# fims9000/SYNT_ISIC

Hardware: AMD Instinct MI355X
Metric: images/sec at 3x64x64 T=1000 (DDPM reverse-diffusion sampling) (higher is better)
Workload: dtype f32

## Files before the change

synt_isic_amd/csrc/common.h:

```cpp
#pragma once

#include <hip/hip_runtime.h>

#include <atomic>
#include <cstdarg>
#include <cstdint>
#include <cstdio>
#include <string>
#include <map>
#include <mutex>
#include <vector>

#include "../../include/sisic.h"

namespace sisic {

void set_error(const char* fmt, ...);

#define SISIC_HIP(call)                                                                   \
    do {                                                                                  \
        hipError_t _e = (call);                                                           \
        if (_e != hipSuccess) {                                                           \
            ::sisic::set_error("%s failed: %s (%s:%d)", #call, hipGetErrorString(_e),     \
                               __FILE__, __LINE__);                                       \
            return SISIC_EHIP;                                                            \
        }                                                                                 \
    } while (0)

#define SISIC_REQUIRE(cond, ...)                 \
    do {                                         \
        if (!(cond)) {                           \
            ::sisic::set_error(__VA_ARGS__);     \
            return SISIC_EINVAL;                 \
        }                                        \
    } while (0)

#define SISIC_TRY(expr)             \
    do {                            \
        int _rc = (expr);           \
        if (_rc != SISIC_OK) return _rc; \
    } while (0)

enum ProfileKind { PK_CONV3 = 0, PK_CONV1 = 1, PK_GN = 2, PK_ATTN = 3, PK_DDPM = 4, PK_OTHER = 5, PK_WINO_MAIN = 6, PK_WINO_BF3 = 7, PK_COUNT = 8 };

struct ProfileSlot {
    double ms = 0, bytes = 0, flops = 0, flops_exec = 0;
    int64_t launches = 0;
};

struct PendingEvent {
    hipEvent_t start, stop;
    int kind;
    int kind2;
};

}

struct sisic_ctx {
    int device = 0;
    int num_cus = 0;
    bool profiling = false;
    sisic::ProfileSlot prof[sisic::PK_COUNT];
    std::vector<sisic::PendingEvent> pending;
    std::vector<hipEvent_t> event_pool;
    struct SplitK { float* p = nullptr; size_t floats = 0; };
    std::map<hipStream_t, SplitK> splitk;
    std::mutex splitk_mutex;
    std::atomic<uint64_t> scratch_generation{0};
};

namespace sisic {

struct ProfileScope {
    sisic_ctx* ctx;
    hipStream_t stream;
    PendingEvent ev{};
    bool active = false;
    ProfileScope(sisic_ctx* c, hipStream_t s, int kind, double bytes, double flops, double flops_exec = -1.0, int kind2 = -1);
    ~ProfileScope();
};

int profile_collect(sisic_ctx* ctx);

inline int ensure_dynamic_lds(sisic_ctx* ctx, const void* kern, int bytes, std::atomic<uint64_t>& done) {
    const uint64_t bit = uint64_t(1) << (ctx->device & 63);
    if (done.load(std::memory_order_acquire) & bit) return SISIC_OK;
    SISIC_HIP(hipFuncSetAttribute(kern, hipFuncAttributeMaxDynamicSharedMemorySize, bytes));
    done.fetch_or(bit, std::memory_order_release);
    return SISIC_OK;
}

inline int cdiv(int a, int b) { return (a + b - 1) / b; }
inline int wino_latency_ksplit(int Cout, int Cin, int Hout, int Wout) {
    const int co_t = Cout > 64 ? 128 : 64;
    const int per_image = cdiv(Hout, 8) * cdiv(Wout, 16) * cdiv(Cout, co_t);
    const int nchunks = cdiv(Cin, 8);
    int k = 1;
    while (per_image * k < 256 && k < 8 && nchunks % (2 * k) == 0) k *= 2;
    return k;
}
inline int wino_latency_segments(int Hout, int Wout) { return cdiv(Hout * Wout, 1024); }
inline int64_t cdiv64(int64_t a, int64_t b) { return (a + b - 1) / b; }
inline int round_up(int a, int b) { return cdiv(a, b) * b; }

constexpr int CONV_CO_TILE = 64;
inline int conv_ci_chunk(int ksize) { return ksize == 1 ? 32 : (ksize == 3 ? 16 : 4); }
inline int conv_cin_pad(int cin, int ksize) { return round_up(cin, conv_ci_chunk(ksize)); }
inline int conv_cout_pad(int cout) { return round_up(cout, CONV_CO_TILE); }
inline int64_t conv_packed_floats(int cout, int cin, int ksize) {
    const int64_t first = (int64_t)conv_cin_pad(cin, ksize) * ksize * ksize * conv_cout_pad(cout);
    return ksize == 1 ? 3 * first + first / 2 : first;
}

int launch_conv2d(sisic_ctx*, const sisic_conv_args& a, hipStream_t s);
int launch_conv_smallcout(sisic_ctx*, const sisic_conv_args& a, hipStream_t s);
int launch_score_head_bwd(sisic_ctx*, const float* logits, const float* fc_w, const float* act, float* g, int B, int C,
                          int HW, int n_classes, int target, hipStream_t s);
int launch_relu_bwd(sisic_ctx*, const float* dy, const float* y, float* out, int64_t n, hipStream_t s);
int launch_scatter_add_even(sisic_ctx*, float* dst, const float* src, int planes, int H, int W, hipStream_t s);
int launch_maxpool_bwd(sisic_ctx*, const float* dm, const float* xin, float* dx, int planes, int H, int W, hipStream_t s);
int launch_stem_bwd(sisic_ctx*, const float* g, const float* w_oihw, float* dp, int B, int CO, int OH, int OW, int H, int W,
                    hipStream_t s);
int launch_preprocess_bwd(sisic_ctx*, const float* dp, const float* x, float* dx, int B, int H, int W, int OH, int OW,
                          hipStream_t s);
int launch_add_relu(sisic_ctx*, const float* y, const float* identity, float* out, int64_t n, hipStream_t s);
int launch_gradcam(sisic_ctx*, const float* y, const float* outp, const float* fc_w, const float* bias, float* cam, int B, int C,
                   int h, int w, int S, int target, hipStream_t s);
int conv_stats_slots(const sisic_conv_args& a);
bool conv_finalizes(const sisic_conv_args& a);
bool conv_pointwise_applicable(const sisic_conv_args& a);
int conv_pointwise_stats_slots(const sisic_conv_args& a);
int launch_conv_pointwise(sisic_ctx*, const sisic_conv_args& a, hipStream_t s);
bool conv_pointwise_bf3_applicable(const sisic_conv_args& a);
int launch_conv_pointwise_bf3(sisic_ctx*, const sisic_conv_args& a, hipStream_t s);
int launch_gn_finalize(sisic_ctx*, const float* st0, int c0, int slots0, const float* st1, int c1, int slots1, int B,
                       int HW, int groups, float eps, const float* gamma, const float* beta, float* scale, float* shift,
                       hipStream_t s, float* mean_rstd = nullptr);
int launch_conv_winograd(sisic_ctx*, const sisic_conv_args& a, const float* u_packed, int cfg, hipStream_t s);
int launch_winograd_pack(sisic_ctx*, const float* w, int Cout, int Cin, float* packed, hipStream_t s);
int64_t winograd_packed_numel(int Cout, int Cin);
inline int64_t winograd_first_floats(int Cout, int Cin) { return (int64_t)round_up(Cin, 16) * 16 * conv_cout_pad(Cout); }
int launch_conv_pack(sisic_ctx*, const float* w, int Cout, int Cin, int k, float* packed, hipStream_t s);
int launch_gn_stats(sisic_ctx*, const float* in0, int c0, const float* in1, int c1, int B, int HW, int groups,
                    float eps, const float* gamma, const float* beta, float* scale, float* shift, hipStream_t s,
                    float* mean_rstd = nullptr);
int launch_attention(sisic_ctx*, const float* qkv, float* out, int B, int C, int N, int head_dim, hipStream_t s);
int launch_ddpm_step(sisic_ctx*, const float* eps, const float* x, const float* z, float* out, int64_t n,
                     float sb, float sa, float c0, float c1, float sigma, float clip, hipStream_t s);
size_t loop_state_bytes();
int launch_loop_select_row(sisic_ctx*, const float* table, int R, const void* state, float* out, hipStream_t s);
int launch_loop_advance(sisic_ctx*, void* state, hipStream_t s);
int launch_ddpm_step_indexed(sisic_ctx*, const float* eps, float* x, int64_t n, const void* state, const float* coef,
                             const int* zrow, float clip, hipStream_t s);
int launch_ddpm_step_rng(sisic_ctx*, const float* eps, const float* x, float* out, int64_t n, int64_t n_per_image,
                         const uint64_t* seeds_dev, uint32_t step, float sb, float sa, float c0, float c1, float sigma,
                         float clip, hipStream_t s);
int launch_ddpm_step_indexed_rng(sisic_ctx*, const float* eps, float* x, int64_t n, int64_t n_per_image, const void* state,
                                 const float* coef, const uint64_t* seeds_dev, float clip, hipStream_t s);
int launch_noise_fill(sisic_ctx*, void* out, int B, int64_t n_per_image, const uint64_t* seeds_host, uint32_t step,
                      uint32_t tag, bool bits, hipStream_t s);
int launch_denorm_u8(sisic_ctx*, const float* x, uint8_t* out, int B, int C, int H, int W, hipStream_t s, int form = 0);
int launch_temb_mlp(sisic_ctx*, const float* t_vals, int B, const float* freqs, int n_freqs, const float* w1t,
                    const float* b1, const float* w2t, const float* b2, int hidden, float* temb_act, hipStream_t s,
                    float* save_emb = nullptr, float* save_h1 = nullptr, float* save_t2 = nullptr);
int launch_linear_t(sisic_ctx*, const float* x, int B, int K, const float* wt, const float* bias, int R,
                    float* out, hipStream_t s);
int launch_transpose2d(sisic_ctx*, const float* in, int rows, int cols, float* out, int out_ld, int out_col0,
                       hipStream_t s);
int launch_preprocess(sisic_ctx*, const float* x, float* out, int B, int H, int W, int OH, int OW, hipStream_t s);
int launch_maxpool(sisic_ctx*, const float* x, float* out, int B, int C, int H, int W, hipStream_t s);
int launch_avgpool_fc(sisic_ctx*, const float* x, const float* w, const float* bias, float* out, int B, int C, int HW,
                      int n_out, hipStream_t s);
int launch_class_scores(sisic_ctx*, const float* logits, int B, int n, int target, float* prob, float* logscore,
                        hipStream_t s);
int launch_mask_patches(sisic_ctx*, const float* image, const uint8_t* masks, float* out, int S, int C, int H, int W,
                        int patch, hipStream_t s);

}
```

synt_isic_amd/csrc/conv_mfma.hip:

```cpp
#include <cstdlib>
#include <type_traits>

#include "common.h"
#include "pack_device.h"

namespace sisic {

typedef float f32x16 __attribute__((ext_vector_type(16)));

struct ConvParams {
    const float* in0;
    const float* in1;
    int c0, c1;
    int B, Hin, Win;
    int Hc, Wc;
    int Hout, Wout;
    int ups;
    int zero_insert;
    const float* w;
    int cout_pad;
    const float* bias;
    int Cout;
    const float* gn_scale;
    const float* gn_shift;
    int gn_silu;
    const float* chan_bias;
    int chan_bias_stride;
    const float* residual;
    int relu;
    float* out;
    float* stats;
    int* slots_query;
    int tiles_x, tiles_y, n_co_tiles, nwg, nchunks;
};

__device__ __forceinline__ float half_wave_sum(float v) {
    v += __int_as_float(__builtin_amdgcn_update_dpp(0, __float_as_int(v), 0xB1, 0xf, 0xf, true));
    v += __int_as_float(__builtin_amdgcn_update_dpp(0, __float_as_int(v), 0x4E, 0xf, 0xf, true));
    v += __int_as_float(__builtin_amdgcn_update_dpp(0, __float_as_int(v), 0x141, 0xf, 0xf, true));
    v += __int_as_float(__builtin_amdgcn_update_dpp(0, __float_as_int(v), 0x140, 0xf, 0xf, true));
    return v + __shfl_xor(v, 16);
}

__device__ __forceinline__ float silu_f(float v) { return v * __builtin_amdgcn_rcpf(1.0f + __expf(-v)); }

template <int KS, int STRIDE, int MT, int NT, int WM, int WN, int TW, int CIC, int KSP = 1>
struct ConvGeom {
    static constexpr int NWAVES = WM * WN * KSP;
    static constexpr int NTHR = 64 * NWAVES;
    static constexpr int CO_TILE = WM * MT * 32;
    static constexpr int PIX = WN * NT * 32;
    static constexpr int TH = PIX / TW;
    static constexpr int KK = KS * KS;
    static constexpr int PAD = KS / 2;
    static constexpr int IH = (TH - 1) * STRIDE + KS;
    static constexpr int IW = (TW - 1) * STRIDE + KS;
    static constexpr int TPC = NTHR / CIC;
    static constexpr int EPT = (IH * IW + TPC - 1) / TPC;
    static constexpr int CHS = EPT * TPC;
    static constexpr int IN_BUF = ((CIC * CHS + 3) / 4) * 4;
    static constexpr int W_F4 = CIC * KK * CO_TILE / 4;
    static constexpr int W_F4_PT = (W_F4 + NTHR - 1) / NTHR;
    static constexpr int W_BUF = W_F4_PT * NTHR * 4;
    static constexpr size_t LDS_BYTES = size_t(2) * (IN_BUF + W_BUF) * sizeof(float);
    static_assert(CO_TILE == CONV_CO_TILE, "weight packing assumes 64-channel tiles");
    static_assert(PIX % TW == 0, "tile must be whole rows");
    static_assert(NTHR % CIC == 0, "staging split");
    static_assert(CIC % (2 * KSP) == 0, "two channels per MFMA, whole pairs per K group");
};

template <int KS, int STRIDE, int MT, int NT, int WM, int WN, int TW, int CIC, int OCC, int KSP, bool V4 = false>
__global__ void __launch_bounds__(64 * WM * WN * KSP, OCC) conv_mfma_kernel(const ConvParams p) {
    using G = ConvGeom<KS, STRIDE, MT, NT, WM, WN, TW, CIC, KSP>;
    static_assert(!V4 || (KS == 1 && STRIDE == 1 && TW == G::PIX && G::EPT % 4 == 0 && G::CHS % 4 == 0),
                  "the float4 staging path is for flat 1x1 tiles");
    extern __shared__ __attribute__((aligned(16))) float smem[];
    float* const in_lds = smem;
    float* const w_lds = smem + 2 * G::IN_BUF;

    int work;
    {
        const int L = blockIdx.x, nwg = p.nwg;
        const int xcd = L & 7, slot = L >> 3, q = nwg >> 3, r = nwg & 7;
        work = (xcd < r ? xcd * (q + 1) : r * (q + 1) + (xcd - r) * q) + slot;
    }
    const int co_t = work % p.n_co_tiles;
    int tile = work / p.n_co_tiles;
    const int tx = tile % p.tiles_x;
    tile /= p.tiles_x;
    const int ty = tile % p.tiles_y;
    const int b = tile / p.tiles_y;
    const int oy0 = ty * G::TH, ox0 = tx * TW;
    const int co0 = co_t * G::CO_TILE;

    const int tid = threadIdx.x;
    const int lane = tid & 63;
    const int wave = tid >> 6;
    const int kg = wave / (WM * WN), wq = wave % (WM * WN);
    const int wm = wq / WN, wn = wq % WN;
    const int half = lane >> 5, l31 = lane & 31;

    const int sci = tid / G::TPC;
    const int sl = tid % G::TPC;
    const int HWin = p.Hin * p.Win;
    const int Cin = p.c0 + p.c1;
    int goff[G::EPT];
    unsigned vmask = 0;
    constexpr int EPT4 = V4 ? G::EPT / 4 : 1;
    int goff4[EPT4];
    unsigned vmask4 = 0;
    if constexpr (V4) {
#pragma unroll
        for (int i = 0; i < EPT4; ++i) {
            const int px = ox0 + 4 * sl + i * G::TPC * 4;
            const bool v = px < p.Wc;
            goff4[i] = v ? px : 0;
            vmask4 |= (v ? 1u : 0u) << i;
        }
    }
#pragma unroll
    for (int i = 0; i < (V4 ? 0 : G::EPT); ++i) {
        const int e = sl + i * G::TPC;
        const int yy = e / G::IW, xx = e % G::IW;
        const int gy = oy0 * STRIDE - G::PAD + yy;
        const int gx = ox0 * STRIDE - G::PAD + xx;
        const bool v = (e < G::IH * G::IW) && gy >= 0 && gy < p.Hc && gx >= 0 && gx < p.Wc &&
                       !(p.zero_insert && ((gy | gx) & 1));
        goff[i] = v ? ((gy >> p.ups) * p.Win + (gx >> p.ups)) : 0;
        vmask |= (v ? 1u : 0u) << i;
    }
    static_assert(G::EPT <= 32, "valid mask is 32 bits");

    const int a_base = half * G::KK * G::CO_TILE + wm * MT * 32 + l31;
    int b_base;
    {
        const int pix = wn * NT * 32 + l31;
        const int y = pix / TW, x = pix % TW;
        b_base = half * G::CHS + (y * STRIDE) * G::IW + x * STRIDE;
    }
    constexpr int NT_STEP = (TW >= 32) ? ((TW > 32) ? 32 * STRIDE : STRIDE * G::IW) : (32 / TW) * STRIDE * G::IW;
    static_assert(TW >= 32 || 32 % TW == 0, "TW must divide 32");
    static_assert(TW <= 32 || TW % 32 == 0, "TW must be a multiple of 32");

    f32x16 acc[MT][NT];
#pragma unroll
    for (int m = 0; m < MT; ++m)
#pragma unroll
        for (int n = 0; n < NT; ++n)
#pragma unroll
            for (int r = 0; r < 16; ++r) acc[m][n][r] = 0.0f;

    float rin[G::EPT];
    float rw[G::W_F4_PT * 4];
    float gsc = 1.0f, gsh = 0.0f;
    bool cval = false;

    const int prologue = (p.gn_scale == nullptr) ? 0 : (p.gn_silu ? 2 : 1);

    auto load_chunk = [&](int chunk) __attribute__((always_inline)) {
        const int c = chunk * CIC + sci;
        cval = c < Cin;
        const int cc = min(c, Cin - 1);
        const float* src = (cc < p.c0) ? p.in0 + ((size_t)b * p.c0 + cc) * HWin
                                       : p.in1 + ((size_t)b * p.c1 + (cc - p.c0)) * HWin;
        if constexpr (V4) {
#pragma unroll
            for (int i = 0; i < EPT4; ++i) {
                const float4 t = *reinterpret_cast<const float4*>(src + goff4[i]);
                rin[4 * i + 0] = t.x; rin[4 * i + 1] = t.y; rin[4 * i + 2] = t.z; rin[4 * i + 3] = t.w;
            }
        } else {
#pragma unroll
            for (int i = 0; i < G::EPT; ++i) rin[i] = src[goff[i]];
        }
        if (prologue) {
            gsc = p.gn_scale[(size_t)b * Cin + cc];
            gsh = p.gn_shift[(size_t)b * Cin + cc];
        }
        const float* wsrc = p.w + (size_t)chunk * CIC * G::KK * p.cout_pad + co0;
#pragma unroll
        for (int i = 0; i < G::W_F4_PT; ++i) {
            const int f = min(tid + i * G::NTHR, G::W_F4 - 1);
            const int rr = f / (G::CO_TILE / 4), c4 = f % (G::CO_TILE / 4);
            const float4 t = *reinterpret_cast<const float4*>(wsrc + (size_t)rr * p.cout_pad + c4 * 4);
            rw[4 * i + 0] = t.x; rw[4 * i + 1] = t.y; rw[4 * i + 2] = t.z; rw[4 * i + 3] = t.w;
        }
    };

    auto store_chunk = [&](const int buf) __attribute__((always_inline)) {
        float* dst = in_lds + buf * G::IN_BUF + sci * G::CHS + sl;
        const unsigned m = cval ? vmask : 0u;
        float v[G::EPT];
        if (prologue == 2) {
#pragma unroll
            for (int i = 0; i < G::EPT; ++i) v[i] = silu_f(rin[i] * gsc + gsh);
        } else if (prologue == 1) {
#pragma unroll
            for (int i = 0; i < G::EPT; ++i) v[i] = rin[i] * gsc + gsh;
        } else {
#pragma unroll
            for (int i = 0; i < G::EPT; ++i) v[i] = rin[i];
        }
        if constexpr (V4) {
            float* dst4 = in_lds + buf * G::IN_BUF + sci * G::CHS + 4 * sl;
            const unsigned m4 = cval ? vmask4 : 0u;
#pragma unroll
            for (int i = 0; i < EPT4; ++i) {
                const bool on = (m4 >> i) & 1u;
                *reinterpret_cast<float4*>(dst4 + i * G::TPC * 4) =
                    make_float4(on ? v[4 * i + 0] : 0.0f, on ? v[4 * i + 1] : 0.0f, on ? v[4 * i + 2] : 0.0f, on ? v[4 * i + 3] : 0.0f);
            }
        } else {
#pragma unroll
            for (int i = 0; i < G::EPT; ++i) dst[i * G::TPC] = ((m >> i) & 1u) ? v[i] : 0.0f;
        }
        float* wdst = w_lds + buf * G::W_BUF + tid * 4;
#pragma unroll
        for (int i = 0; i < G::W_F4_PT; ++i)
            *reinterpret_cast<float4*>(wdst + i * G::NTHR * 4) =
                make_float4(rw[4 * i + 0], rw[4 * i + 1], rw[4 * i + 2], rw[4 * i + 3]);
    };

    auto compute_chunk = [&](const int buf) __attribute__((always_inline)) {
        const float* A = w_lds + buf * G::W_BUF + a_base;
        const float* Bm = in_lds + buf * G::IN_BUF + b_base;
#pragma unroll
        for (int cp = kg * (CIC / 2 / KSP); cp < (kg + 1) * (CIC / 2 / KSP); ++cp) {
#pragma unroll
            for (int ky = 0; ky < KS; ++ky) {
#pragma unroll
                for (int kx = 0; kx < KS; ++kx) {
                    float a[MT], bb[NT];
#pragma unroll
                    for (int m = 0; m < MT; ++m)
                        a[m] = A[(2 * cp * G::KK + ky * KS + kx) * G::CO_TILE + m * 32];
#pragma unroll
                    for (int n = 0; n < NT; ++n)
                        bb[n] = Bm[2 * cp * G::CHS + ky * G::IW + kx + n * NT_STEP];
#pragma unroll
                    for (int m = 0; m < MT; ++m)
#pragma unroll
                        for (int n = 0; n < NT; ++n)
                            acc[m][n] = __builtin_amdgcn_mfma_f32_32x32x2f32(a[m], bb[n], acc[m][n], 0, 0, 0);
                }
            }
        }
    };

    load_chunk(0);
    store_chunk(0);
    __syncthreads();
    auto step = [&](const int chunk, auto buf_tag) __attribute__((always_inline)) {
        constexpr int BUF = decltype(buf_tag)::value;
        const bool more = chunk + 1 < p.nchunks;
        if (more) load_chunk(chunk + 1);
        compute_chunk(BUF);
        if (more) store_chunk(BUF ^ 1);
        __syncthreads();
    };
    {
        int chunk = 0;
        for (; chunk + 1 < p.nchunks; chunk += 2) {
            step(chunk, std::integral_constant<int, 0>{});
            step(chunk + 1, std::integral_constant<int, 1>{});
        }
        if (chunk < p.nchunks) step(chunk, std::integral_constant<int, 0>{});
    }

    if constexpr (KSP > 1) {
        static_assert(KSP == 2, "two K groups");
        static_assert((size_t)WM * WN * MT * NT * 16 * 64 * sizeof(float) <= G::LDS_BYTES, "reduction slab fits the staging LDS");
        float* red = smem + (size_t)wq * MT * NT * 16 * 64 + lane;
        if (kg == 1) {
#pragma unroll
            for (int m = 0; m < MT; ++m)
#pragma unroll
                for (int n = 0; n < NT; ++n)
#pragma unroll
                    for (int r = 0; r < 16; ++r) red[((m * NT + n) * 16 + r) * 64] = acc[m][n][r];
        }
        __syncthreads();
        if (kg != 0) return;
#pragma unroll
        for (int m = 0; m < MT; ++m)
#pragma unroll
            for (int n = 0; n < NT; ++n)
#pragma unroll
                for (int r = 0; r < 16; ++r) acc[m][n][r] += red[((m * NT + n) * 16 + r) * 64];
    }

    const size_t HWout = (size_t)p.Hout * p.Wout;
    float cbias[MT][16];
#pragma unroll
    for (int m = 0; m < MT; ++m) {
#pragma unroll
        for (int r = 0; r < 16; ++r) {
            cbias[m][r] = 0.0f;
        }
    }
    if (p.bias) {
#pragma unroll
        for (int m = 0; m < MT; ++m)
#pragma unroll
            for (int r = 0; r < 16; ++r)
                cbias[m][r] += p.bias[min(co0 + wm * MT * 32 + m * 32 + (r & 3) + 8 * (r >> 2) + 4 * half, p.Cout - 1)];
    }
    if (p.chan_bias) {
        const float* cb = p.chan_bias + (size_t)b * p.chan_bias_stride;
#pragma unroll
        for (int m = 0; m < MT; ++m)
#pragma unroll
            for (int r = 0; r < 16; ++r)
                cbias[m][r] += cb[min(co0 + wm * MT * 32 + m * 32 + (r & 3) + 8 * (r >> 2) + 4 * half, p.Cout - 1)];
    }
    float psum[MT][16];
#pragma unroll
    for (int m = 0; m < MT; ++m)
#pragma unroll
        for (int r = 0; r < 16; ++r) psum[m][r] = 0.0f;
    unsigned pvmask = 0;
#pragma unroll
    for (int n = 0; n < NT; ++n) {
        const int pix = wn * NT * 32 + n * 32 + l31;
        const int oy = oy0 + pix / TW, ox = ox0 + pix % TW;
        const bool pv = oy < p.Hout && ox < p.Wout;
        pvmask |= pv ? (1u << n) : 0u;
        const size_t pix_off = (size_t)min(oy, p.Hout - 1) * p.Wout + min(ox, p.Wout - 1);
#pragma unroll
        for (int m = 0; m < MT; ++m) {
            float res[16];
#pragma unroll
            for (int r = 0; r < 16; ++r) res[r] = 0.0f;
            if (p.residual) {
#pragma unroll
                for (int r = 0; r < 16; ++r) {
                    const int co = min(co0 + wm * MT * 32 + m * 32 + (r & 3) + 8 * (r >> 2) + 4 * half, p.Cout - 1);
                    res[r] = p.residual[((size_t)b * p.Cout + co) * HWout + pix_off];
                }
            }
#pragma unroll
            for (int r = 0; r < 16; ++r) {
                const int co = co0 + wm * MT * 32 + m * 32 + (r & 3) + 8 * (r >> 2) + 4 * half;
                float v = acc[m][n][r] + cbias[m][r] + res[r];
                if (p.relu) v = fmaxf(v, 0.0f);
                if (pv && co < p.Cout) p.out[((size_t)b * p.Cout + co) * HWout + pix_off] = v;
                acc[m][n][r] = v;
                psum[m][r] += pv ? v : 0.0f;
            }
        }
    }

    if (p.stats) {
        const float cnt = half_wave_sum((float)__builtin_popcount(pvmask));
        const float inv = 1.0f / fmaxf(cnt, 1.0f);
        const int slots = p.tiles_x * p.tiles_y * WN, slot = (ty * p.tiles_x + tx) * WN + wn;
#pragma unroll
        for (int m = 0; m < MT; ++m) {
#pragma unroll
            for (int r = 0; r < 16; ++r) {
                const int co = co0 + wm * MT * 32 + m * 32 + (r & 3) + 8 * (r >> 2) + 4 * half;
                const float s1 = half_wave_sum(psum[m][r]);
                const float mean = s1 * inv;
                float q = 0.0f;
#pragma unroll
                for (int n = 0; n < NT; ++n) {
                    const float d = acc[m][n][r] - mean;
                    q += ((pvmask >> n) & 1u) ? d * d : 0.0f;
                }
                q = half_wave_sum(q);
                if (l31 == 0 && co < p.Cout)
                    reinterpret_cast<float4*>(p.stats)[((size_t)b * p.Cout + co) * slots + slot] = make_float4(cnt, s1, q, 0.0f);
            }
        }
    }
}


__global__ void conv_pack_kernel(const float* __restrict__ w, int Cout, int Cin, int KK, int cin_pad, int cout_pad,
                                 float* __restrict__ out) {
    const size_t first = (size_t)cin_pad * KK * cout_pad;
    const size_t total = KK == 1 ? 3 * first + first / 2 : first;
    for (size_t i = (size_t)blockIdx.x * blockDim.x + threadIdx.x; i < total; i += (size_t)gridDim.x * blockDim.x) {
        conv_pack_elem(i, w, Cout, Cin, KK, cin_pad, cout_pad, out);
    }
}

template <int KS, int STRIDE, int MT, int NT, int WM, int WN, int TW, int CIC, int OCC = 2, int KSP = 1>
static int launch_cfg(sisic_ctx* ctx, ConvParams& p, hipStream_t s) {
    using G = ConvGeom<KS, STRIDE, MT, NT, WM, WN, TW, CIC, KSP>;
    p.tiles_x = cdiv(p.Wout, TW);
    p.tiles_y = cdiv(p.Hout, G::TH);
    p.n_co_tiles = p.cout_pad / G::CO_TILE;
    p.nchunks = cdiv(p.c0 + p.c1, CIC);
    const int64_t nwg = (int64_t)p.B * p.tiles_x * p.tiles_y * p.n_co_tiles;
    SISIC_REQUIRE(nwg > 0 && nwg < (int64_t(1) << 31), "conv2d: grid of %lld workgroups unsupported", (long long)nwg);
    p.nwg = (int)nwg;
    if (p.slots_query) {
        *p.slots_query = p.tiles_x * p.tiles_y * WN;
        return SISIC_OK;
    }
    if constexpr (KS == 1 && STRIDE == 1 && TW == G::PIX && G::EPT % 4 == 0) {
        const bool aligned = ((reinterpret_cast<uintptr_t>(p.in0) | reinterpret_cast<uintptr_t>(p.in1)) & 15) == 0;
        if (p.Wc % 4 == 0 && aligned) {
            auto kern4 = conv_mfma_kernel<KS, STRIDE, MT, NT, WM, WN, TW, CIC, OCC, KSP, true>;
            static std::atomic<uint64_t> lds_opt_in4{0};
            SISIC_TRY(ensure_dynamic_lds(ctx, reinterpret_cast<const void*>(kern4), (int)G::LDS_BYTES, lds_opt_in4));
            hipLaunchKernelGGL(kern4, dim3(p.nwg), dim3(G::NTHR), G::LDS_BYTES, s, p);
            SISIC_HIP(hipGetLastError());
            return SISIC_OK;
        }
    }
    auto kern = conv_mfma_kernel<KS, STRIDE, MT, NT, WM, WN, TW, CIC, OCC, KSP>;
    static std::atomic<uint64_t> lds_opt_in{0};
    SISIC_TRY(ensure_dynamic_lds(ctx, reinterpret_cast<const void*>(kern), (int)G::LDS_BYTES, lds_opt_in));
    hipLaunchKernelGGL(kern, dim3(p.nwg), dim3(G::NTHR), G::LDS_BYTES, s, p);
    SISIC_HIP(hipGetLastError());
    return SISIC_OK;
}

int launch_conv_pack(sisic_ctx*, const float* w, int Cout, int Cin, int k, float* packed, hipStream_t s) {
    SISIC_REQUIRE(k == 1 || k == 3 || k == 7, "conv_pack: ksize %d unsupported", k);
    const int cin_pad = conv_cin_pad(Cin, k), cout_pad = conv_cout_pad(Cout);
    const size_t total = (size_t)cin_pad * k * k * cout_pad;
    const int blocks = (int)std::min<size_t>((total * (k == 1 ? 4 : 1) + 255) / 256, 4096);
    hipLaunchKernelGGL(conv_pack_kernel, dim3(blocks), dim3(256), 0, s, w, Cout, Cin, k * k, cin_pad, cout_pad, packed);
    SISIC_HIP(hipGetLastError());
    return SISIC_OK;
}

static int dispatch_conv2d(sisic_ctx* ctx, const sisic_conv_args& a, hipStream_t s, int* slots_query);

static int winograd_cfg(const sisic_conv_args& a) {
    if (!(a.ksize == 3 && a.stride == 1 && a.w_winograd != nullptr && a.Cout > 4) || a.upsample == 2) return 0;
    if ((a.tile_cfg >= 60 && a.tile_cfg <= 74) || a.tile_cfg == 78 || a.tile_cfg == 79 || (a.tile_cfg >= 90 && a.tile_cfg <= 92)) return a.tile_cfg;
    if (a.tile_cfg != 0) return 0;
    const int Hout = a.Hin << (a.upsample ? 1 : 0), Wout = a.Win << (a.upsample ? 1 : 0);
    const bool fits32 = 16.0 * std::max(a.c0, a.c1) * a.Hin * a.Win < 4294967296.0;
    if (!fits32) return 0;
    if (Hout >= 12 && Wout >= 12) {
        static const bool wide_on = [] { const char* e = std::getenv("SISIC_WINO_WIDE"); return !e || std::atoi(e) != 0; }();
        static const bool bf3_on = [] { const char* e = std::getenv("SISIC_WINO_BF16X3"); return !e || std::atoi(e) != 0; }();
        const int th = (Hout + 15) / 16 * 16, tw = (Wout + 15) / 16 * 16;
        if (bf3_on && a.Cout % 64 == 0 && 4 * Hout * Wout >= 3 * th * tw && a.c0 + a.c1 >= 16 &&
            a.c0 + a.c1 <= 2048 &&
            4.0 * a.Cout * Hout * Wout < 2147483648.0)
            return 74;
        if (wide_on && !a.upsample) return a.Cout > 64 ? 68 : 69;
        return 66;
    }
    const int Cin = a.c0 + a.c1;
    static const bool ksplit_on = [] { const char* e = std::getenv("SISIC_KSPLIT"); return !e || std::atoi(e) != 0; }();
    if (ksplit_on && Hout <= 8 && Wout <= 8 && Hout >= 5 && Wout >= 5 && Cin >= 128 && Cin % 32 == 0 && a.Cout >= 128) {
        static const bool wide_on = [] { const char* e = std::getenv("SISIC_WINO_WIDE"); return !e || std::atoi(e) != 0; }();
        static const bool bf3_on = [] { const char* e = std::getenv("SISIC_WINO_BF16X3"); return !e || std::atoi(e) != 0; }();
        if (bf3_on && !a.upsample && a.Cout % 64 == 0 && Cin <= 512) return 92;
        return (wide_on && !a.upsample) ? 91 : 90;
    }
    return 0;
}
static bool winograd_selected(const sisic_conv_args& a) { return winograd_cfg(a) != 0; }

int conv_stats_slots(const sisic_conv_args& a) {
    if (const int cfg = winograd_cfg(a)) {
        if (cfg >= 90 && cfg <= 92) return 1;
        const int Hout = a.Hin << (a.upsample ? 1 : 0), Wout = a.Win << (a.upsample ? 1 : 0);
        if ((cfg == 78 || cfg == 79) && wino_latency_ksplit(a.Cout, a.c0 + a.c1, Hout, Wout) > 1) return wino_latency_segments(Hout, Wout);
        if ((cfg >= 68 && cfg <= 73) || cfg == 78 || cfg == 79) return ((Hout + 7) / 8) * ((Wout + 15) / 16);
        const int edge = (cfg == 61 || cfg == 63 || cfg == 65 || cfg == 67) ? 8 : 16;
        return ((Hout + edge - 1) / edge) * ((Wout + edge - 1) / edge);
    }
    int slots = 0;
    sisic_conv_args q = a;
    q.stats_out = nullptr;
    if (dispatch_conv2d(nullptr, q, nullptr, &slots) != SISIC_OK) return 0;
    return slots;
}

bool conv_finalizes(const sisic_conv_args& a) {
    if (!a.fin_gamma || a.fin_groups <= 0) return false;
    const int cfg = winograd_cfg(a);
    const int Hout = a.Hin << (a.upsample ? 1 : 0), Wout = a.Win << (a.upsample ? 1 : 0);
    if (a.Cout % a.fin_groups != 0 || a.Cout / a.fin_groups != 8) return false;
    if (cfg == 74) return !a.upsample && Hout <= 16 && Wout <= 16 && a.Cout % 64 == 0;
    if (cfg < 90 || cfg > 92) return false;
    if (Hout * Wout != 64 || a.Cout % 16 != 0) return false;
    return ((reinterpret_cast<uintptr_t>(a.residual) | reinterpret_cast<uintptr_t>(a.out) | reinterpret_cast<uintptr_t>(a.stats_out)) & 15) == 0;
}

int launch_conv2d(sisic_ctx* ctx, const sisic_conv_args& a, hipStream_t s) { return dispatch_conv2d(ctx, a, s, nullptr); }

static int dispatch_conv2d(sisic_ctx* ctx, const sisic_conv_args& a, hipStream_t s, int* slots_query) {
    SISIC_REQUIRE(a.in0 && a.w_packed && a.out, "conv2d: null tensor");
    SISIC_REQUIRE(a.B > 0 && a.Hin > 0 && a.Win > 0 && a.c0 > 0 && a.c1 >= 0 && a.Cout > 0, "conv2d: bad shape");
    SISIC_REQUIRE((a.c1 == 0) == (a.in1 == nullptr), "conv2d: in1/c1 mismatch");
    SISIC_REQUIRE(a.ksize == 1 || a.ksize == 3 || a.ksize == 7, "conv2d: ksize %d unsupported", a.ksize);
    SISIC_REQUIRE(a.stride == 1 || a.stride == 2, "conv2d: stride %d unsupported", a.stride);
    SISIC_REQUIRE(a.ksize != 7 || a.stride == 2, "conv2d: 7x7 is built for stride 2 only (the ResNet stem)");
    SISIC_REQUIRE(!(a.upsample && a.stride != 1), "conv2d: upsample with stride");
    SISIC_REQUIRE((a.gn_scale == nullptr) == (a.gn_shift == nullptr), "conv2d: gn_scale/gn_shift mismatch");

    ConvParams p{};
    p.in0 = a.in0; p.in1 = a.in1; p.c0 = a.c0; p.c1 = a.c1;
    p.B = a.B; p.Hin = a.Hin; p.Win = a.Win;
    p.ups = a.upsample ? 1 : 0;
    p.zero_insert = a.upsample == 2 ? 1 : 0;
    p.Hc = a.Hin << p.ups; p.Wc = a.Win << p.ups;
    const int pad = a.ksize / 2;
    p.Hout = (p.Hc + 2 * pad - a.ksize) / a.stride + 1;
    p.Wout = (p.Wc + 2 * pad - a.ksize) / a.stride + 1;
    p.w = a.w_packed; p.cout_pad = conv_cout_pad(a.Cout);
    p.bias = a.bias; p.Cout = a.Cout;
    p.gn_scale = a.gn_scale; p.gn_shift = a.gn_shift; p.gn_silu = a.gn_silu;
    p.chan_bias = a.chan_bias; p.chan_bias_stride = a.chan_bias_stride; p.residual = a.residual; p.relu = a.relu; p.out = a.out;
    p.stats = a.stats_out; p.slots_query = slots_query;

    const int Cin = a.c0 + a.c1;
    const double kk = double(a.ksize) * a.ksize;
    const double out_elems = double(a.B) * a.Cout * p.Hout * p.Wout;
    const double bytes = 4.0 * (double(a.B) * Cin * a.Hin * a.Win + out_elems) + 4.0 * (Cin * a.Cout * kk + a.Cout) +
                         (a.residual ? 4.0 * out_elems : 0.0);
    const double flops = 2.0 * out_elems * Cin * kk;
    int cfg = a.tile_cfg;
    const bool use_wino = winograd_selected(a);
    SISIC_REQUIRE(a.stats_out == nullptr || conv_stats_slots(a) > 0,
                  "conv2d: stats_out given but sisic_conv_stats_slots() is 0 for these arguments");
    const bool wino_ups9 = use_wino && a.upsample && !a.gn_scale && winograd_cfg(a) == 66;
    ProfileScope prof(slots_query ? nullptr : ctx, s, a.ksize == 1 ? PK_CONV1 : PK_CONV3, bytes, flops,
                      use_wino ? flops * (wino_ups9 ? 9.0 : 16.0) / 36.0 : flops,
                      (use_wino && winograd_cfg(a) == 74) ? PK_WINO_BF3 :
                      (use_wino && !wino_ups9 && (winograd_cfg(a) == 66 || (winograd_cfg(a) >= 68 && winograd_cfg(a) <= 73) || winograd_cfg(a) == 78 || winograd_cfg(a) == 79)) ? PK_WINO_MAIN : -1);

    if (a.ksize == 3 && a.stride == 1 && !a.upsample && a.Cout <= 4 && (cfg == 0 || (cfg >= 50 && cfg <= 52))) {
        if (slots_query) return SISIC_OK;
        return launch_conv_smallcout(ctx, a, s);
    }
    if (use_wino) {
        SISIC_REQUIRE(!slots_query, "conv2d: internal: slot query on the Winograd path");
        return launch_conv_winograd(ctx, a, a.w_winograd, winograd_cfg(a), s);
    }
    SISIC_REQUIRE((cfg < 60 || cfg > 74) && cfg != 78 && cfg != 79 && (cfg < 90 || cfg > 92), "conv2d: tile_cfg %d needs w_winograd, ksize 3 and stride 1", cfg);
    if (a.ksize == 7) {
        if (cfg == 0) cfg = 41;
        if (cfg == 41) return launch_cfg<7, 2, 2, 1, 1, 4, 32, 2>(ctx, p, s);
        if (cfg == 42) return launch_cfg<7, 2, 2, 1, 1, 4, 32, 4>(ctx, p, s);
    } else if (a.ksize == 1 && a.stride == 2) {
        if (cfg == 0) cfg = p.Wout >= 24 ? 31 : (p.Wout >= 12 ? 32 : 33);
        switch (cfg) {
            case 31: return launch_cfg<1, 2, 2, 1, 1, 4, 32, 16>(ctx, p, s);
            case 32: return launch_cfg<1, 2, 2, 1, 1, 4, 16, 16>(ctx, p, s);
            case 33: return launch_cfg<1, 2, 1, 1, 2, 2, 8, 16>(ctx, p, s);
        }
    } else if (a.ksize == 1) {
        p.Hin = 1; p.Win = a.Hin * a.Win; p.Hc = 1; p.Wc = p.Win; p.Hout = 1; p.Wout = p.Win; p.ups = 0;
        SISIC_REQUIRE(!a.upsample, "conv2d: 1x1 with upsample");
        static const bool pw_on = [] { const char* e = std::getenv("SISIC_POINTWISE"); return !e || std::atoi(e) != 0; }();
        static const bool pwb_on = [] { const char* e = std::getenv("SISIC_POINTWISE_BF16X3"); return !e || std::atoi(e) != 0; }();
        if ((cfg == 0 && pwb_on && conv_pointwise_bf3_applicable(a)) || (cfg >= 28 && cfg <= 30) || cfg == 34 || cfg == 35) {
            if (slots_query) { *slots_query = conv_pointwise_stats_slots(a); return SISIC_OK; }
            return launch_conv_pointwise_bf3(ctx, a, s);
        }
        if ((cfg == 0 && pw_on && conv_pointwise_applicable(a)) || cfg == 20) {
            if (slots_query) { *slots_query = conv_pointwise_stats_slots(a); return SISIC_OK; }
            return launch_conv_pointwise(ctx, a, s);
        }
        if (cfg == 0) cfg = (p.Wout <= 64) ? 22 : (p.Wout <= 256 ? 25 : 24);
        switch (cfg) {
            case 21: return launch_cfg<1, 1, 2, 2, 1, 4, 256, 16>(ctx, p, s);
            case 22: return launch_cfg<1, 1, 1, 1, 2, 2, 64, 16>(ctx, p, s);
            case 23: return launch_cfg<1, 1, 2, 1, 1, 4, 128, 16>(ctx, p, s);
            case 24: return launch_cfg<1, 1, 1, 2, 2, 4, 256, 32, 4>(ctx, p, s);
            case 25: return launch_cfg<1, 1, 1, 1, 2, 4, 128, 32, 4>(ctx, p, s);
            case 26: return launch_cfg<1, 1, 1, 2, 2, 4, 256, 16, 4>(ctx, p, s);
            case 27: return launch_cfg<1, 1, 1, 1, 2, 4, 128, 16, 4>(ctx, p, s);
        }
    } else if (a.stride == 1) {
        if (cfg == 0) cfg = p.Wout >= 24 ? 8 : (p.Wout >= 12 ? 9 : 16);
        switch (cfg) {
            case 1: return launch_cfg<3, 1, 2, 2, 1, 4, 64, 8>(ctx, p, s);
            case 2: return launch_cfg<3, 1, 2, 2, 1, 4, 32, 8>(ctx, p, s);
            case 3: return launch_cfg<3, 1, 2, 2, 1, 4, 16, 8>(ctx, p, s);
            case 4: return launch_cfg<3, 1, 1, 1, 2, 2, 8, 8>(ctx, p, s);
            case 16: return launch_cfg<3, 1, 1, 1, 2, 2, 8, 16, 2, 2>(ctx, p, s);
            case 17: return launch_cfg<3, 1, 1, 1, 2, 2, 8, 8, 2, 2>(ctx, p, s);
            case 5: return launch_cfg<3, 1, 2, 1, 1, 4, 16, 8>(ctx, p, s);
            case 6: return launch_cfg<3, 1, 2, 1, 1, 4, 64, 8>(ctx, p, s);
            case 7: return launch_cfg<3, 1, 2, 1, 1, 4, 32, 8>(ctx, p, s);
            case 8: return launch_cfg<3, 1, 1, 2, 2, 4, 32, 8, 4>(ctx, p, s);
            case 9: return launch_cfg<3, 1, 1, 2, 2, 4, 16, 8, 4>(ctx, p, s);
            case 10: return launch_cfg<3, 1, 1, 2, 2, 4, 32, 8, 2>(ctx, p, s);
            case 14: return launch_cfg<3, 1, 1, 1, 2, 4, 16, 8, 4>(ctx, p, s);
            case 15: return launch_cfg<3, 1, 1, 1, 2, 4, 8, 8, 4>(ctx, p, s);
        }
    } else {
        if (cfg == 0) cfg = p.Wout >= 24 ? 11 : (p.Wout >= 12 ? 12 : 18);
        switch (cfg) {
            case 11: return launch_cfg<3, 2, 2, 1, 1, 4, 32, 8>(ctx, p, s);
            case 12: return launch_cfg<3, 2, 2, 1, 1, 4, 16, 8>(ctx, p, s);
            case 13: return launch_cfg<3, 2, 1, 1, 2, 2, 8, 8>(ctx, p, s);
            case 18: return launch_cfg<3, 2, 1, 1, 2, 2, 8, 16, 2, 2>(ctx, p, s);
            case 19: return launch_cfg<3, 2, 1, 1, 2, 2, 8, 8, 2, 2>(ctx, p, s);
        }
    }
    set_error("conv2d: tile_cfg %d invalid for ksize %d stride %d", cfg, a.ksize, a.stride);
    return SISIC_EINVAL;
}

}
```

synt_isic_amd/csrc/conv_pointwise_bf3.hip:

```cpp
#include <cstdlib>
#include <type_traits>

#include "common.h"

namespace sisic {

typedef float pwb_f32x16 __attribute__((ext_vector_type(16)));
typedef short pwb_bf16x8 __attribute__((ext_vector_type(8)));
typedef unsigned pwb_u4 __attribute__((ext_vector_type(4)));
typedef unsigned pwb_u2 __attribute__((ext_vector_type(2)));
typedef float pwb_f2 __attribute__((ext_vector_type(2)));
typedef float pwb_f4 __attribute__((ext_vector_type(4)));

struct PwbParams {
    const float* in0;
    const float* in1;
    int c0, c1, B, HW;
    const float* wb;
    int n_co64;
    const float* bias;
    int Cout;
    const float* gn_scale;
    const float* gn_shift;
    const float* chan_bias;
    int chan_bias_stride;
    const float* residual;
    int relu;
    float* out;
    float* stats;
    int n_px, n_co_items, nitems, nwg, nchunks;
};

constexpr int PWB_WAVES = 4;

__device__ __forceinline__ float pwb_half_wave_sum(float v) {
    v += __int_as_float(__builtin_amdgcn_update_dpp(0, __float_as_int(v), 0xB1, 0xf, 0xf, true));
    v += __int_as_float(__builtin_amdgcn_update_dpp(0, __float_as_int(v), 0x4E, 0xf, 0xf, true));
    v += __int_as_float(__builtin_amdgcn_update_dpp(0, __float_as_int(v), 0x141, 0xf, 0xf, true));
    v += __int_as_float(__builtin_amdgcn_update_dpp(0, __float_as_int(v), 0x140, 0xf, 0xf, true));
    return v + __shfl_xor(v, 16);
}
__device__ __forceinline__ float pwb_row16_sum(float v) {
    v += __int_as_float(__builtin_amdgcn_update_dpp(0, __float_as_int(v), 0xB1, 0xf, 0xf, true));
    v += __int_as_float(__builtin_amdgcn_update_dpp(0, __float_as_int(v), 0x4E, 0xf, 0xf, true));
    v += __int_as_float(__builtin_amdgcn_update_dpp(0, __float_as_int(v), 0x141, 0xf, 0xf, true));
    v += __int_as_float(__builtin_amdgcn_update_dpp(0, __float_as_int(v), 0x140, 0xf, 0xf, true));
    return v;
}
__device__ __forceinline__ float pwb_silu(float v) { return v * __builtin_amdgcn_rcpf(1.0f + __expf(-v)); }

template <int PRO, int NB>
__global__ void __launch_bounds__(64 * PWB_WAVES, 4) conv_pwb_kernel(const PwbParams p) {
    extern __shared__ __attribute__((aligned(16))) float smem[];
    int wg;
    {
        const int L = blockIdx.x, nwg = p.nwg;
        const int xcd = L & 7, slot = L >> 3, q = nwg >> 3, r = nwg & 7;
        wg = (xcd < r ? xcd * (q + 1) : r * (q + 1) + (xcd - r) * q) + slot;
    }
    const int tid = threadIdx.x, lane = tid & 63;
    const int wave_u = __builtin_amdgcn_readfirstlane(tid >> 6);
    const int item = wg * PWB_WAVES + wave_u;
    if (item >= p.nitems) return;
    const int half = lane >> 5, l31 = lane & 31;
    int co_i = item % p.n_co_items;
    const int t = item / p.n_co_items;
    int px_t = t % p.n_px, b = t / p.n_px;
    asm volatile("" : "+s"(co_i), "+s"(px_t), "+s"(b));
    constexpr int CB = 2;
    const int px0 = 32 * NB * px_t, co0 = 64 * co_i;
    const int Cin = p.c0 + p.c1, HW = p.HW, n = p.nchunks;

    const __amdgpu_buffer_rsrc_t rs0 = __builtin_amdgcn_make_buffer_rsrc(const_cast<float*>(p.in0 + (size_t)b * p.c0 * HW), 0, -1, 0x00020000);
    const __amdgpu_buffer_rsrc_t rs1 = __builtin_amdgcn_make_buffer_rsrc(
        const_cast<float*>(p.in1 ? p.in1 + (size_t)b * p.c1 * HW : p.in0), 0, -1, 0x00020000);
    const __amdgpu_buffer_rsrc_t rsw = __builtin_amdgcn_make_buffer_rsrc(const_cast<float*>(p.wb), 0, -1, 0x00020000);

    const unsigned x_voff = 4u * (unsigned)((4 * half) * HW + px0 + NB * l31);
    const unsigned a_lane16 = 16u * (unsigned)lane, a_lane8 = 8u * (unsigned)lane;

    float* const gnL = smem + wave_u * (2 * Cin);
    if constexpr (PRO != 0) {
        for (int i = lane; i < Cin; i += 64) {
            gnL[2 * i] = p.gn_scale[(size_t)b * Cin + i];
            gnL[2 * i + 1] = p.gn_shift[(size_t)b * Cin + i];
        }
        asm volatile("s_waitcnt lgkmcnt(0)" ::: "memory");
        __builtin_amdgcn_wave_barrier();
    }

    pwb_f32x16 acc[CB][NB];
#pragma unroll
    for (int x = 0; x < CB; ++x)
#pragma unroll
        for (int nb = 0; nb < NB; ++nb)
#pragma unroll
            for (int r = 0; r < 16; ++r) acc[x][nb][r] = 0.0f;

    struct XRegs {
        pwb_f2 x[4];
    };
    auto ld = [&](const __amdgpu_buffer_rsrc_t rs, unsigned soff) {
        if constexpr (NB == 2) return __builtin_bit_cast(pwb_f2, __builtin_amdgcn_raw_buffer_load_b64(rs, x_voff, soff, 0));
        else return pwb_f2{__builtin_bit_cast(float, __builtin_amdgcn_raw_buffer_load_b32(rs, x_voff, soff, 0)), 0.0f};
    };
    pwb_u4 ua[CB];
    pwb_u2 ul[CB];
    pwb_u4 ub[CB];
    pwb_u2 um[CB];
    auto load_x = [&](int c, XRegs& r) {
#ifdef PWB_DIAG_NO_X_LOADS
        if (c > 1) return;
#endif
        const int cc0 = 8 * c;
        if (cc0 < p.c0) {
            const unsigned soff = 4u * (unsigned)(cc0 * HW);
#pragma unroll
            for (int k = 0; k < 4; ++k)
                r.x[k] = ld(rs0, soff + 4u * (unsigned)(k * HW));
        } else {
            const unsigned soff = 4u * (unsigned)((cc0 - p.c0) * HW);
#pragma unroll
            for (int k = 0; k < 4; ++k)
                r.x[k] = ld(rs1, soff + 4u * (unsigned)(k * HW));
        }
    };
    auto load_a = [&](int c) {
#ifdef PWB_DIAG_NO_FILTER_LOADS
        if (c > 1) return;
#endif
        const unsigned s0 = 3072u * (unsigned)(c * p.n_co64 + co_i);
#pragma unroll
        for (int x = 0; x < CB; ++x) {
            ua[x] = __builtin_amdgcn_raw_buffer_load_b128(rsw, a_lane16, s0 + 1024u * (unsigned)x, 0);
            ul[x] = __builtin_amdgcn_raw_buffer_load_b64(rsw, a_lane8, s0 + 2048u + 512u * (unsigned)x, 0);
        }
    };
    auto load_b = [&](int c) {
#ifdef PWB_DIAG_NO_FILTER_LOADS
        if (c > 1) return;
#endif
        const unsigned s0 = 3072u * (unsigned)(c * p.n_co64 + co_i);
#pragma unroll
        for (int x = 0; x < CB; ++x) {
            ub[x] = __builtin_amdgcn_raw_buffer_load_b128(rsw, a_lane16, s0 + 1024u * (unsigned)x, 0);
            um[x] = __builtin_amdgcn_raw_buffer_load_b64(rsw, a_lane8, s0 + 2048u + 512u * (unsigned)x, 0);
        }
    };
    struct Tup { pwb_u4 hm, mh, lh; };
    auto make = [&](int c, const XRegs& r, int nb) {
        pwb_f4 g01 = {1.0f, 0.0f, 1.0f, 0.0f}, g23 = g01;
        if constexpr (PRO != 0) {
            const float* gp = gnL + 2 * (8 * c + 4 * half);
            g01 = *reinterpret_cast<const pwb_f4*>(gp);
            g23 = *reinterpret_cast<const pwb_f4*>(gp + 4);
        }
        float v[4];
#pragma unroll
        for (int k = 0; k < 4; ++k) {
            float e = nb ? r.x[k].y : r.x[k].x;
            if constexpr (PRO != 0) {
                const float sc = k == 0 ? g01.x : (k == 1 ? g01.z : (k == 2 ? g23.x : g23.z));
                const float sh = k == 0 ? g01.y : (k == 1 ? g01.w : (k == 2 ? g23.y : g23.w));
                e = e * sc + sh;
                if constexpr (PRO == 2) e = pwb_silu(e);
            }
            v[k] = e;
        }
        unsigned hi[2], mid[2], lo[2];
#pragma unroll
        for (int q = 0; q < 2; ++q) {
            const float v0 = v[2 * q], v1 = v[2 * q + 1];
            const unsigned h0 = __float_as_uint(v0) & 0xffff0000u, h1 = __float_as_uint(v1) & 0xffff0000u;
            const float r0 = v0 - __uint_as_float(h0), r1 = v1 - __uint_as_float(h1);
            const unsigned m0 = __float_as_uint(r0) & 0xffff0000u, m1 = __float_as_uint(r1) & 0xffff0000u;
            const float l0 = r0 - __uint_as_float(m0), l1 = r1 - __uint_as_float(m1);
            hi[q] = __builtin_amdgcn_perm(h1, h0, 0x07060302u);
            mid[q] = __builtin_amdgcn_perm(m1, m0, 0x07060302u);
            lo[q] = __builtin_amdgcn_perm(__float_as_uint(l1), __float_as_uint(l0), 0x07060302u);
        }
        return Tup{pwb_u4{hi[0], hi[1], mid[0], mid[1]}, pwb_u4{mid[0], mid[1], hi[0], hi[1]}, pwb_u4{lo[0], lo[1], hi[0], hi[1]}};
    };
    auto mm_with = [&](const Tup& t, auto nb_tag, const pwb_u4 (&fa)[CB], const pwb_u2 (&fl)[CB]) {
        constexpr int nb = decltype(nb_tag)::value;
#pragma unroll
        for (int x = 0; x < CB; ++x) {
            const pwb_u4 a_hl = {fa[x].x, fa[x].y, fl[x].x, fl[x].y};
            acc[x][nb] = __builtin_amdgcn_mfma_f32_32x32x16_bf16(__builtin_bit_cast(pwb_bf16x8, fa[x]), __builtin_bit_cast(pwb_bf16x8, t.hm), acc[x][nb], 0, 0, 0);
            acc[x][nb] = __builtin_amdgcn_mfma_f32_32x32x16_bf16(__builtin_bit_cast(pwb_bf16x8, fa[x]), __builtin_bit_cast(pwb_bf16x8, t.mh), acc[x][nb], 0, 0, 0);
            acc[x][nb] = __builtin_amdgcn_mfma_f32_32x32x16_bf16(__builtin_bit_cast(pwb_bf16x8, a_hl), __builtin_bit_cast(pwb_bf16x8, t.lh), acc[x][nb], 0, 0, 0);
        }
    };
    auto mm = [&](const Tup& t, auto nb_tag) { mm_with(t, nb_tag, ua, ul); };
    using Z = std::integral_constant<int, 0>;
    using O = std::integral_constant<int, 1>;

    XRegs ra, rb;
    load_x(0, ra);
    load_a(0);
    if constexpr (NB == 2) {
        auto compute = [&](int c, const XRegs& r) {
            mm(make(c, r, 0), Z{});
            mm(make(c, r, 1), O{});
        };
        int c = 0;
        for (; c + 1 < n; c += 2) {
            load_x(c + 1, rb);
            compute(c, ra);
            load_a(c + 1);
            if (c + 2 < n) load_x(c + 2, ra);
            compute(c + 1, rb);
            if (c + 2 < n) load_a(c + 2);
        }
        if (c < n) compute(c, ra);
    } else {
        auto weave = [&]() {
#pragma unroll
            for (int i = 0; i < 6; ++i) {
                __builtin_amdgcn_sched_group_barrier(0x008, 1, 0);
                __builtin_amdgcn_sched_group_barrier(0x002, 8, 0);
            }
        };
        if (n > 1) { load_x(1, rb); load_b(1); }
        Tup t = make(0, ra, 0);
        int c = 0;
        for (; c + 2 < n; c += 2) {
            load_x(c + 2, ra);
            Tup u = make(c + 1, rb, 0);
            mm_with(t, Z{}, ua, ul);
            weave();
            load_a(c + 2);
            if (c + 3 < n) load_x(c + 3, rb);
            t = make(c + 2, ra, 0);
            mm_with(u, Z{}, ub, um);
            weave();
            if (c + 3 < n) load_b(c + 3);
        }
        if (c + 1 < n) {
            Tup u = make(c + 1, rb, 0);
            mm_with(t, Z{}, ua, ul);
            mm_with(u, Z{}, ub, um);
        } else {
            mm_with(t, Z{}, ua, ul);
        }
    }

    const __amdgpu_buffer_rsrc_t rso = __builtin_amdgcn_make_buffer_rsrc(p.out + (size_t)b * p.Cout * HW, 0, -1, 0x00020000);
    const __amdgpu_buffer_rsrc_t rsr = __builtin_amdgcn_make_buffer_rsrc(
        const_cast<float*>(p.residual ? p.residual + (size_t)b * p.Cout * HW : p.out), 0, -1, 0x00020000);
    const unsigned o_voff = 4u * (unsigned)((4 * half) * HW + px0 + NB * l31);
    const int slots = HW / 32;
#pragma unroll
    for (int x = 0; x < CB; ++x) {
        float add[16];
        pwb_f2 res[16];
#pragma unroll
        for (int r = 0; r < 16; ++r) {
            const int cs = co0 + 32 * x + 8 * (r >> 2) + (r & 3);
            const int col = cs + 4 * half;
            add[r] = 0.0f;
            if (p.bias) add[r] += p.bias[col];
            if (p.chan_bias) add[r] += p.chan_bias[(size_t)b * p.chan_bias_stride + col];
            res[r] = pwb_f2{0.0f, 0.0f};
            if (p.residual) {
                if constexpr (NB == 2) res[r] = __builtin_bit_cast(pwb_f2, __builtin_amdgcn_raw_buffer_load_b64(rsr, o_voff, 4u * (unsigned)(cs * HW), 0));
                else res[r].x = __builtin_bit_cast(float, __builtin_amdgcn_raw_buffer_load_b32(rsr, o_voff, 4u * (unsigned)(cs * HW), 0));
            }
        }
#pragma unroll
        for (int r = 0; r < 16; ++r) {
            const int cs = co0 + 32 * x + 8 * (r >> 2) + (r & 3);
            float vv[2] = {0.0f, 0.0f};
#pragma unroll
            for (int nb = 0; nb < NB; ++nb) {
                vv[nb] = acc[x][nb][r] + add[r] + (nb ? res[r].y : res[r].x);
                if (p.relu) vv[nb] = fmaxf(vv[nb], 0.0f);
            }
            if constexpr (NB == 2) __builtin_amdgcn_raw_buffer_store_b64(pwb_u2{__float_as_uint(vv[0]), __float_as_uint(vv[1])}, rso, o_voff, 4u * (unsigned)(cs * HW), 0);
            else __builtin_amdgcn_raw_buffer_store_b32(__float_as_uint(vv[0]), rso, o_voff, 4u * (unsigned)(cs * HW), 0);
            if (p.stats) {
                const int co = cs + 4 * half;
                if constexpr (NB == 1) {
                    const float s1 = pwb_half_wave_sum(vv[0]);
                    const float d = vv[0] - s1 * (1.0f / 32.0f);
                    float dd;
                    asm volatile("v_mul_f32 %0, %1, %1" : "=v"(dd) : "v"(d));
                    const float q = pwb_half_wave_sum(dd);
                    if (l31 == 0)
                        reinterpret_cast<float4*>(p.stats)[((size_t)b * p.Cout + co) * slots + px_t] = make_float4(32.0f, s1, q, 0.0f);
                } else {
                    const float s1 = pwb_row16_sum(vv[0] + vv[1]);
                    const float mean = s1 * (1.0f / 32.0f);
                    const float d0 = vv[0] - mean, d1 = vv[1] - mean;
                    float q0, q1;
                    asm volatile("v_mul_f32 %0, %2, %2\n\tv_mul_f32 %1, %3, %3" : "=&v"(q0), "=&v"(q1) : "v"(d0), "v"(d1));
                    const float q = pwb_row16_sum(q0 + q1);
                    if ((l31 & 15) == 0)
                        reinterpret_cast<float4*>(p.stats)[((size_t)b * p.Cout + co) * slots + 2 * px_t + (l31 >> 4)] = make_float4(32.0f, s1, q, 0.0f);
                }
            }
        }
    }
}

#ifndef PWBK_VAR
#define PWBK_VAR 0
#endif
template <int PRO>
__global__ void __launch_bounds__(64 * PWB_WAVES, 4) conv_pwbk_kernel(const PwbParams p) {
    extern __shared__ __attribute__((aligned(16))) float smem[];
    int item;
    {
        const int L = blockIdx.x, nwg = p.nwg;
        const int xcd = L & 7, slot = L >> 3, q = nwg >> 3, r = nwg & 7;
        item = (xcd < r ? xcd * (q + 1) : r * (q + 1) + (xcd - r) * q) + slot;
    }
    const int tid = threadIdx.x, lane = tid & 63;
    const int wave_u = __builtin_amdgcn_readfirstlane(tid >> 6);
    const int half = lane >> 5, l31 = lane & 31;
    int co_i = item % p.n_co_items;
    const int t = item / p.n_co_items;
    int px_t = t % p.n_px, b = t / p.n_px;
    asm volatile("" : "+s"(co_i), "+s"(px_t), "+s"(b));
    constexpr int CB = 2;
    const int px0 = 32 * px_t, co0 = 64 * co_i;
    const int Cin = p.c0 + p.c1, HW = p.HW;
    const int nl = p.nchunks / PWB_WAVES, cb = wave_u * nl;

    const __amdgpu_buffer_rsrc_t rs0 = __builtin_amdgcn_make_buffer_rsrc(const_cast<float*>(p.in0 + (size_t)b * p.c0 * HW), 0, -1, 0x00020000);
    const __amdgpu_buffer_rsrc_t rs1 = __builtin_amdgcn_make_buffer_rsrc(
        const_cast<float*>(p.in1 ? p.in1 + (size_t)b * p.c1 * HW : p.in0), 0, -1, 0x00020000);
    const __amdgpu_buffer_rsrc_t rsw = __builtin_amdgcn_make_buffer_rsrc(const_cast<float*>(p.wb), 0, -1, 0x00020000);
    const unsigned x_voff = 4u * (unsigned)((4 * half) * HW + px0 + l31);
    const unsigned a_lane16 = 16u * (unsigned)lane, a_lane8 = 8u * (unsigned)lane;

    float* const P_lds = smem;
    float* const gnL = smem + PWB_WAVES * 32 * 64 + wave_u * (2 * 8 * nl);
    if constexpr (PRO != 0) {
        for (int i = lane; i < 8 * nl; i += 64) {
            gnL[2 * i] = p.gn_scale[(size_t)b * Cin + 8 * cb + i];
            gnL[2 * i + 1] = p.gn_shift[(size_t)b * Cin + 8 * cb + i];
        }
        asm volatile("s_waitcnt lgkmcnt(0)" ::: "memory");
        __builtin_amdgcn_wave_barrier();
    }

    pwb_f32x16 acc[CB];
#pragma unroll
    for (int x = 0; x < CB; ++x)
#pragma unroll
        for (int r = 0; r < 16; ++r) acc[x][r] = 0.0f;
    struct XRegs { float x[4]; };
    auto load_x = [&](int c, XRegs& r) {
        const int cc0 = 8 * c;
        if (cc0 < p.c0) {
            const unsigned soff = 4u * (unsigned)(cc0 * HW);
#pragma unroll
            for (int k = 0; k < 4; ++k) r.x[k] = __builtin_bit_cast(float, __builtin_amdgcn_raw_buffer_load_b32(rs0, x_voff, soff + 4u * (unsigned)(k * HW), 0));
        } else {
            const unsigned soff = 4u * (unsigned)((cc0 - p.c0) * HW);
#pragma unroll
            for (int k = 0; k < 4; ++k) r.x[k] = __builtin_bit_cast(float, __builtin_amdgcn_raw_buffer_load_b32(rs1, x_voff, soff + 4u * (unsigned)(k * HW), 0));
        }
    };
    auto load_f = [&](int c, pwb_u4 (&fa)[CB], pwb_u2 (&fl)[CB]) {
        const unsigned s0 = 3072u * (unsigned)(c * p.n_co64 + co_i);
#pragma unroll
        for (int x = 0; x < CB; ++x) {
            fa[x] = __builtin_amdgcn_raw_buffer_load_b128(rsw, a_lane16, s0 + 1024u * (unsigned)x, 0);
#if (PWBK_VAR & 1) != 0
            fl[x] = pwb_u2{fa[x].z, fa[x].w};
#else
            fl[x] = __builtin_amdgcn_raw_buffer_load_b64(rsw, a_lane8, s0 + 2048u + 512u * (unsigned)x, 0);
#endif
#if (PWBK_VAR & 2) != 0
            fa[x] = pwb_u4{a_lane16 + (unsigned)c, a_lane8, s0, a_lane16 ^ s0};
            fl[x] = pwb_u2{fa[x].z, fa[x].w};
#endif
        }
    };
    struct Tup { pwb_u4 hm, mh, lh; };
    auto make = [&](int cl, const XRegs& r) {
        pwb_f4 g01 = {1.0f, 0.0f, 1.0f, 0.0f}, g23 = g01;
        if constexpr (PRO != 0) {
            const float* gp = gnL + 2 * (8 * cl + 4 * half);
            g01 = *reinterpret_cast<const pwb_f4*>(gp);
            g23 = *reinterpret_cast<const pwb_f4*>(gp + 4);
        }
        float v[4];
#pragma unroll
        for (int k = 0; k < 4; ++k) {
            float e = r.x[k];
            if constexpr (PRO != 0) {
                const float sc = k == 0 ? g01.x : (k == 1 ? g01.z : (k == 2 ? g23.x : g23.z));
                const float sh = k == 0 ? g01.y : (k == 1 ? g01.w : (k == 2 ? g23.y : g23.w));
                e = e * sc + sh;
                if constexpr (PRO == 2) e = pwb_silu(e);
            }
            v[k] = e;
        }
        unsigned hi[2], mid[2], lo[2];
#pragma unroll
        for (int q = 0; q < 2; ++q) {
            const float v0 = v[2 * q], v1 = v[2 * q + 1];
            const unsigned h0 = __float_as_uint(v0) & 0xffff0000u, h1 = __float_as_uint(v1) & 0xffff0000u;
            const float r0 = v0 - __uint_as_float(h0), r1 = v1 - __uint_as_float(h1);
            const unsigned m0 = __float_as_uint(r0) & 0xffff0000u, m1 = __float_as_uint(r1) & 0xffff0000u;
            const float l0 = r0 - __uint_as_float(m0), l1 = r1 - __uint_as_float(m1);
            hi[q] = __builtin_amdgcn_perm(h1, h0, 0x07060302u);
            mid[q] = __builtin_amdgcn_perm(m1, m0, 0x07060302u);
            lo[q] = __builtin_amdgcn_perm(__float_as_uint(l1), __float_as_uint(l0), 0x07060302u);
        }
        return Tup{pwb_u4{hi[0], hi[1], mid[0], mid[1]}, pwb_u4{mid[0], mid[1], hi[0], hi[1]}, pwb_u4{lo[0], lo[1], hi[0], hi[1]}};
    };
    auto mm = [&](const Tup& t, const pwb_u4 (&fa)[CB], const pwb_u2 (&fl)[CB]) {
#pragma unroll
        for (int x = 0; x < CB; ++x) {
            const pwb_u4 a_hl = {fa[x].x, fa[x].y, fl[x].x, fl[x].y};
            acc[x] = __builtin_amdgcn_mfma_f32_32x32x16_bf16(__builtin_bit_cast(pwb_bf16x8, fa[x]), __builtin_bit_cast(pwb_bf16x8, t.hm), acc[x], 0, 0, 0);
            acc[x] = __builtin_amdgcn_mfma_f32_32x32x16_bf16(__builtin_bit_cast(pwb_bf16x8, fa[x]), __builtin_bit_cast(pwb_bf16x8, t.mh), acc[x], 0, 0, 0);
            acc[x] = __builtin_amdgcn_mfma_f32_32x32x16_bf16(__builtin_bit_cast(pwb_bf16x8, a_hl), __builtin_bit_cast(pwb_bf16x8, t.lh), acc[x], 0, 0, 0);
        }
    };
    constexpr int XD = 4;
    XRegs xr[XD];
    pwb_u4 ua[CB], ub[CB];
    pwb_u2 ul[CB], um[CB];
#pragma unroll
    for (int i = 0; i < XD; ++i)
        if (i < nl) load_x(cb + i, xr[i]);
    load_f(cb, ua, ul);
    if (nl > 1) load_f(cb + 1, ub, um);
    for (int c = 0; c < nl; c += XD) {
#pragma unroll
        for (int i = 0; i < XD; ++i) {
            if (c + i < nl) {
                const Tup t = make(c + i, xr[i]);
                if (c + i + XD < nl) load_x(cb + c + i + XD, xr[i]);
                if ((i & 1) == 0) {
                    mm(t, ua, ul);
                    if (c + i + 2 < nl) load_f(cb + c + i + 2, ua, ul);
                } else {
                    mm(t, ub, um);
                    if (c + i + 2 < nl) load_f(cb + c + i + 2, ub, um);
                }
            }
        }
    }

#pragma unroll
    for (int x = 0; x < CB; ++x)
#pragma unroll
        for (int r = 0; r < 16; ++r) P_lds[((wave_u * 2 + x) * 16 + r) * 64 + lane] = acc[x][r];
    __syncthreads();
    const int x = wave_u >> 1, rb = 8 * (wave_u & 1);
    const __amdgpu_buffer_rsrc_t rso = __builtin_amdgcn_make_buffer_rsrc(p.out + (size_t)b * p.Cout * HW, 0, -1, 0x00020000);
    const __amdgpu_buffer_rsrc_t rsr = __builtin_amdgcn_make_buffer_rsrc(
        const_cast<float*>(p.residual ? p.residual + (size_t)b * p.Cout * HW : p.out), 0, -1, 0x00020000);
    const unsigned o_voff = 4u * (unsigned)((4 * half) * HW + px0 + l31);
    const int slots = HW / 32;
    float add[8], res[8];
#pragma unroll
    for (int rr = 0; rr < 8; ++rr) {
        const int r = rb + rr;
        const int cs = co0 + 32 * x + 8 * (r >> 2) + (r & 3);
        const int col = cs + 4 * half;
        add[rr] = 0.0f;
        if (p.bias) add[rr] += p.bias[col];
        if (p.chan_bias) add[rr] += p.chan_bias[(size_t)b * p.chan_bias_stride + col];
        res[rr] = 0.0f;
        if (p.residual) res[rr] = __builtin_bit_cast(float, __builtin_amdgcn_raw_buffer_load_b32(rsr, o_voff, 4u * (unsigned)(cs * HW), 0));
    }
#pragma unroll
    for (int rr = 0; rr < 8; ++rr) {
        const int r = rb + rr;
        const int cs = co0 + 32 * x + 8 * (r >> 2) + (r & 3);
        float part[PWB_WAVES];
#pragma unroll
        for (int k = 0; k < PWB_WAVES; ++k) part[k] = P_lds[((k * 2 + x) * 16 + r) * 64 + lane];
        float v = ((part[0] + part[1]) + part[2]) + part[3];
        v = v + add[rr] + res[rr];
        if (p.relu) v = fmaxf(v, 0.0f);
        __builtin_amdgcn_raw_buffer_store_b32(__float_as_uint(v), rso, o_voff, 4u * (unsigned)(cs * HW), 0);
        if (p.stats) {
            const int co = cs + 4 * half;
            const float s1 = pwb_half_wave_sum(v);
            const float d = v - s1 * (1.0f / 32.0f);
            float dd;
            asm volatile("v_mul_f32 %0, %1, %1" : "=v"(dd) : "v"(d));
            const float q = pwb_half_wave_sum(dd);
            if (l31 == 0)
                reinterpret_cast<float4*>(p.stats)[((size_t)b * p.Cout + co) * slots + px_t] = make_float4(32.0f, s1, q, 0.0f);
        }
    }
}

constexpr int PWBS_MAX_WAVES = 12;
template <int PRO>
__global__ void __launch_bounds__(64 * PWBS_MAX_WAVES) conv_pwbs_kernel(const PwbParams p) {
    extern __shared__ __attribute__((aligned(16))) float smem[];
    int wg;
    {
        const int L = blockIdx.x, nwg = p.nwg;
        const int xcd = L & 7, slot = L >> 3, q = nwg >> 3, r = nwg & 7;
        wg = (xcd < r ? xcd * (q + 1) : r * (q + 1) + (xcd - r) * q) + slot;
    }
    const int tid = threadIdx.x, lane = tid & 63;
    const int wave_u = __builtin_amdgcn_readfirstlane(tid >> 6);
    const int nwaves = p.n_co_items;
    const int half = lane >> 5, l31 = lane & 31;
    int px_t = wg % p.n_px, b = wg / p.n_px;
    asm volatile("" : "+s"(px_t), "+s"(b));
    constexpr int CB = 2, NB = 2;
    const int co_i = wave_u;
    const int px0 = 64 * px_t, co0 = 64 * co_i;
    const int Cin = p.c0 + p.c1, HW = p.HW, n = p.nchunks;

    const __amdgpu_buffer_rsrc_t rs0 = __builtin_amdgcn_make_buffer_rsrc(const_cast<float*>(p.in0 + (size_t)b * p.c0 * HW), 0, -1, 0x00020000);
    const __amdgpu_buffer_rsrc_t rs1 = __builtin_amdgcn_make_buffer_rsrc(
        const_cast<float*>(p.in1 ? p.in1 + (size_t)b * p.c1 * HW : p.in0), 0, -1, 0x00020000);
    const __amdgpu_buffer_rsrc_t rsw = __builtin_amdgcn_make_buffer_rsrc(const_cast<float*>(p.wb), 0, -1, 0x00020000);
    const unsigned x_voff = 4u * (unsigned)((4 * half) * HW + px0 + NB * l31);
    const unsigned a_lane16 = 16u * (unsigned)lane, a_lane8 = 8u * (unsigned)lane;

    unsigned* const S_hm = reinterpret_cast<unsigned*>(smem);
    unsigned* const S_lo = S_hm + (size_t)n * NB * 64 * 4;
    float* const gnL = reinterpret_cast<float*>(S_lo + (size_t)n * NB * 64 * 2);
    if constexpr (PRO != 0) {
        for (int i = tid; i < Cin; i += 64 * nwaves) {
            gnL[2 * i] = p.gn_scale[(size_t)b * Cin + i];
            gnL[2 * i + 1] = p.gn_shift[(size_t)b * Cin + i];
        }
        __syncthreads();
    }
    for (int c = wave_u; c < n; c += nwaves) {
        pwb_f2 xr[4];
        const int cc0 = 8 * c;
        if (cc0 < p.c0) {
            const unsigned soff = 4u * (unsigned)(cc0 * HW);
#pragma unroll
            for (int k = 0; k < 4; ++k) xr[k] = __builtin_bit_cast(pwb_f2, __builtin_amdgcn_raw_buffer_load_b64(rs0, x_voff, soff + 4u * (unsigned)(k * HW), 0));
        } else {
            const unsigned soff = 4u * (unsigned)((cc0 - p.c0) * HW);
#pragma unroll
            for (int k = 0; k < 4; ++k) xr[k] = __builtin_bit_cast(pwb_f2, __builtin_amdgcn_raw_buffer_load_b64(rs1, x_voff, soff + 4u * (unsigned)(k * HW), 0));
        }
        pwb_f4 g01 = {1.0f, 0.0f, 1.0f, 0.0f}, g23 = g01;
        if constexpr (PRO != 0) {
            const float* gp = gnL + 2 * (8 * c + 4 * half);
            g01 = *reinterpret_cast<const pwb_f4*>(gp);
            g23 = *reinterpret_cast<const pwb_f4*>(gp + 4);
        }
#pragma unroll
        for (int nb = 0; nb < NB; ++nb) {
            float v[4];
#pragma unroll
            for (int k = 0; k < 4; ++k) {
                float e = nb ? xr[k].y : xr[k].x;
                if constexpr (PRO != 0) {
                    const float sc = k == 0 ? g01.x : (k == 1 ? g01.z : (k == 2 ? g23.x : g23.z));
                    const float sh = k == 0 ? g01.y : (k == 1 ? g01.w : (k == 2 ? g23.y : g23.w));
                    e = e * sc + sh;
                    if constexpr (PRO == 2) e = pwb_silu(e);
                }
                v[k] = e;
            }
            unsigned hi[2], mid[2], lo[2];
#pragma unroll
            for (int q = 0; q < 2; ++q) {
                const float v0 = v[2 * q], v1 = v[2 * q + 1];
                const unsigned h0 = __float_as_uint(v0) & 0xffff0000u, h1 = __float_as_uint(v1) & 0xffff0000u;
                const float r0 = v0 - __uint_as_float(h0), r1 = v1 - __uint_as_float(h1);
                const unsigned m0 = __float_as_uint(r0) & 0xffff0000u, m1 = __float_as_uint(r1) & 0xffff0000u;
                const float l0 = r0 - __uint_as_float(m0), l1 = r1 - __uint_as_float(m1);
                hi[q] = __builtin_amdgcn_perm(h1, h0, 0x07060302u);
                mid[q] = __builtin_amdgcn_perm(m1, m0, 0x07060302u);
                lo[q] = __builtin_amdgcn_perm(__float_as_uint(l1), __float_as_uint(l0), 0x07060302u);
            }
            *reinterpret_cast<pwb_u4*>(S_hm + ((size_t)(c * NB + nb) * 64 + lane) * 4) = pwb_u4{hi[0], hi[1], mid[0], mid[1]};
            *reinterpret_cast<pwb_u2*>(S_lo + ((size_t)(c * NB + nb) * 64 + lane) * 2) = pwb_u2{lo[0], lo[1]};
        }
    }
    __syncthreads();

    pwb_f32x16 acc[CB][NB];
#pragma unroll
    for (int x = 0; x < CB; ++x)
#pragma unroll
        for (int nb = 0; nb < NB; ++nb)
#pragma unroll
            for (int r = 0; r < 16; ++r) acc[x][nb][r] = 0.0f;
    pwb_u4 ua[CB], ub[CB];
    pwb_u2 ul[CB], um[CB];
    auto load_f = [&](int c, pwb_u4 (&fa)[CB], pwb_u2 (&fl)[CB]) {
        const unsigned s0 = 3072u * (unsigned)(c * p.n_co64 + co_i);
#pragma unroll
        for (int x = 0; x < CB; ++x) {
            fa[x] = __builtin_amdgcn_raw_buffer_load_b128(rsw, a_lane16, s0 + 1024u * (unsigned)x, 0);
            fl[x] = __builtin_amdgcn_raw_buffer_load_b64(rsw, a_lane8, s0 + 2048u + 512u * (unsigned)x, 0);
        }
    };
    auto chunk = [&](int c, const pwb_u4 (&fa)[CB], const pwb_u2 (&fl)[CB]) {
#pragma unroll
        for (int nb = 0; nb < NB; ++nb) {
            const pwb_u4 hm = *reinterpret_cast<const pwb_u4*>(S_hm + ((size_t)(c * NB + nb) * 64 + lane) * 4);
            const pwb_u2 lo = *reinterpret_cast<const pwb_u2*>(S_lo + ((size_t)(c * NB + nb) * 64 + lane) * 2);
            const pwb_u4 mh = {hm.z, hm.w, hm.x, hm.y}, lh = {lo.x, lo.y, hm.x, hm.y};
#pragma unroll
            for (int x = 0; x < CB; ++x) {
                const pwb_u4 a_hl = {fa[x].x, fa[x].y, fl[x].x, fl[x].y};
                acc[x][nb] = __builtin_amdgcn_mfma_f32_32x32x16_bf16(__builtin_bit_cast(pwb_bf16x8, fa[x]), __builtin_bit_cast(pwb_bf16x8, hm), acc[x][nb], 0, 0, 0);
                acc[x][nb] = __builtin_amdgcn_mfma_f32_32x32x16_bf16(__builtin_bit_cast(pwb_bf16x8, fa[x]), __builtin_bit_cast(pwb_bf16x8, mh), acc[x][nb], 0, 0, 0);
                acc[x][nb] = __builtin_amdgcn_mfma_f32_32x32x16_bf16(__builtin_bit_cast(pwb_bf16x8, a_hl), __builtin_bit_cast(pwb_bf16x8, lh), acc[x][nb], 0, 0, 0);
            }
        }
    };
    load_f(0, ua, ul);
    if (n > 1) load_f(1, ub, um);
    {
        int c = 0;
        for (; c + 1 < n; c += 2) {
            chunk(c, ua, ul);
            if (c + 2 < n) load_f(c + 2, ua, ul);
            chunk(c + 1, ub, um);
            if (c + 3 < n) load_f(c + 3, ub, um);
        }
        if (c < n) chunk(c, ua, ul);
    }

    const __amdgpu_buffer_rsrc_t rso = __builtin_amdgcn_make_buffer_rsrc(p.out + (size_t)b * p.Cout * HW, 0, -1, 0x00020000);
    const __amdgpu_buffer_rsrc_t rsr = __builtin_amdgcn_make_buffer_rsrc(
        const_cast<float*>(p.residual ? p.residual + (size_t)b * p.Cout * HW : p.out), 0, -1, 0x00020000);
    const unsigned o_voff = 4u * (unsigned)((4 * half) * HW + px0 + NB * l31);
    const int slots = HW / 32;
#pragma unroll
    for (int x = 0; x < CB; ++x) {
        float add[16];
        pwb_f2 res[16];
#pragma unroll
        for (int r = 0; r < 16; ++r) {
            const int cs = co0 + 32 * x + 8 * (r >> 2) + (r & 3);
            const int col = cs + 4 * half;
            add[r] = 0.0f;
            if (p.bias) add[r] += p.bias[col];
            if (p.chan_bias) add[r] += p.chan_bias[(size_t)b * p.chan_bias_stride + col];
            res[r] = pwb_f2{0.0f, 0.0f};
            if (p.residual) res[r] = __builtin_bit_cast(pwb_f2, __builtin_amdgcn_raw_buffer_load_b64(rsr, o_voff, 4u * (unsigned)(cs * HW), 0));
        }
#pragma unroll
        for (int r = 0; r < 16; ++r) {
            const int cs = co0 + 32 * x + 8 * (r >> 2) + (r & 3);
            float vv[2];
#pragma unroll
            for (int nb = 0; nb < NB; ++nb) {
                vv[nb] = acc[x][nb][r] + add[r] + (nb ? res[r].y : res[r].x);
                if (p.relu) vv[nb] = fmaxf(vv[nb], 0.0f);
            }
            __builtin_amdgcn_raw_buffer_store_b64(pwb_u2{__float_as_uint(vv[0]), __float_as_uint(vv[1])}, rso, o_voff, 4u * (unsigned)(cs * HW), 0);
            if (p.stats) {
                const int co = cs + 4 * half;
                const float s1 = pwb_row16_sum(vv[0] + vv[1]);
                const float mean = s1 * (1.0f / 32.0f);
                const float d0 = vv[0] - mean, d1 = vv[1] - mean;
                float q0, q1;
                asm volatile("v_mul_f32 %0, %2, %2\n\tv_mul_f32 %1, %3, %3" : "=&v"(q0), "=&v"(q1) : "v"(d0), "v"(d1));
                const float q = pwb_row16_sum(q0 + q1);
                if ((l31 & 15) == 0)
                    reinterpret_cast<float4*>(p.stats)[((size_t)b * p.Cout + co) * slots + 2 * px_t + (l31 >> 4)] = make_float4(32.0f, s1, q, 0.0f);
            }
        }
    }
}

static bool pwbk_on() { static const bool on = [] { const char* e = std::getenv("SISIC_POINTWISE_KSPLIT"); return !e || std::atoi(e) != 0; }(); return on; }
template <int PRO>
static int launch_pwbk(sisic_ctx* ctx, PwbParams& p, int Cin, hipStream_t s) {
    p.n_co_items = p.Cout / 64;
    p.n_px = p.HW / 32;
    const int64_t nitems = (int64_t)p.B * p.n_px * p.n_co_items;
    SISIC_REQUIRE(nitems > 0 && nitems < (int64_t(1) << 31), "conv2d(pointwise bf16x3, K-split): grid too large");
    p.nitems = (int)nitems;
    p.nwg = p.nitems;
    const size_t lds = sizeof(float) * (size_t)(PWB_WAVES * 32 * 64 + (PRO ? 2 * Cin : 0));
    static std::atomic<uint64_t> opt{0};
    auto kern = conv_pwbk_kernel<PRO>;
    SISIC_TRY(ensure_dynamic_lds(ctx, reinterpret_cast<const void*>(kern), (int)lds, opt));
    hipLaunchKernelGGL(kern, dim3(p.nwg), dim3(64 * PWB_WAVES), lds, s, p);
    SISIC_HIP(hipGetLastError());
    return SISIC_OK;
}

static size_t pwbs_lds_bytes(int Cin) { return (size_t)(Cin / 8) * 2 * 64 * 24 + 8 * (size_t)Cin; }
static bool pwbs_applicable(const sisic_conv_args& a) {
    const int items = a.Cout / 64;
    return items >= 6 && items <= PWBS_MAX_WAVES && pwbs_lds_bytes(a.c0 + a.c1) <= 150 * 1024;
}
template <int PRO>
static int launch_pwbs(sisic_ctx* ctx, PwbParams& p, int Cin, hipStream_t s) {
    p.n_co_items = p.Cout / 64;
    p.n_px = p.HW / 64;
    const int64_t nwg = (int64_t)p.B * p.n_px;
    SISIC_REQUIRE(nwg > 0 && nwg < (int64_t(1) << 31), "conv2d(pointwise bf16x3, staged): grid too large");
    p.nwg = (int)nwg;
    p.nitems = p.nwg * p.n_co_items;
    const size_t lds = pwbs_lds_bytes(Cin);
    static std::atomic<uint64_t> opt{0};
    auto kern = conv_pwbs_kernel<PRO>;
    SISIC_TRY(ensure_dynamic_lds(ctx, reinterpret_cast<const void*>(kern), (int)lds, opt));
    hipLaunchKernelGGL(kern, dim3(p.nwg), dim3(64 * p.n_co_items), lds, s, p);
    SISIC_HIP(hipGetLastError());
    return SISIC_OK;
}

bool conv_pointwise_bf3_applicable(const sisic_conv_args& a) {
    if (a.ksize != 1 || a.stride != 1 || a.upsample) return false;
    const int HW = a.Hin * a.Win, Cin = a.c0 + a.c1;
    if (HW % 64 != 0 || Cin % 8 != 0 || (a.c1 != 0 && a.c0 % 8 != 0) || a.Cout % 64 != 0) return false;
    if (((reinterpret_cast<uintptr_t>(a.in0) | reinterpret_cast<uintptr_t>(a.in1) | reinterpret_cast<uintptr_t>(a.out) |
          reinterpret_cast<uintptr_t>(a.residual)) & 7) != 0) return false;
    if (4.0 * std::max(std::max(a.c0, a.c1), a.Cout) * HW >= 4294967296.0 || 6.0 * conv_cin_pad(Cin, 1) * conv_cout_pad(a.Cout) >= 4294967296.0) return false;
    if (a.gn_scale && Cin > 1024) return false;
    return true;
}

template <int PRO, int NB>
static int launch_pwb(sisic_ctx* ctx, PwbParams& p, int Cin, hipStream_t s) {
    p.n_co_items = p.Cout / 64;
    p.n_px = p.HW / (32 * NB);
    const int64_t nitems = (int64_t)p.B * p.n_px * p.n_co_items;
    SISIC_REQUIRE(nitems > 0 && nitems < (int64_t(1) << 31), "conv2d(pointwise bf16x3): grid too large");
    p.nitems = (int)nitems;
    p.nwg = (int)((nitems + PWB_WAVES - 1) / PWB_WAVES);
    const size_t lds = PRO ? sizeof(float) * (size_t)(PWB_WAVES * 2 * Cin) : 0;
    static std::atomic<uint64_t> opt{0};
    auto kern = conv_pwb_kernel<PRO, NB>;
    SISIC_TRY(ensure_dynamic_lds(ctx, reinterpret_cast<const void*>(kern), (int)lds, opt));
    hipLaunchKernelGGL(kern, dim3(p.nwg), dim3(64 * PWB_WAVES), lds, s, p);
    SISIC_HIP(hipGetLastError());
    return SISIC_OK;
}

int launch_conv_pointwise_bf3(sisic_ctx* ctx, const sisic_conv_args& a, hipStream_t s) {
    SISIC_REQUIRE(conv_pointwise_bf3_applicable(a), "conv2d(pointwise bf16x3): shape not supported by tile_cfg 28");
    PwbParams p{};
    const int Cin = a.c0 + a.c1;
    p.in0 = a.in0; p.in1 = a.in1; p.c0 = a.c0; p.c1 = a.c1; p.B = a.B; p.HW = a.Hin * a.Win;
    p.wb = a.w_packed + 2 * (size_t)conv_cin_pad(Cin, 1) * conv_cout_pad(a.Cout);
    p.n_co64 = conv_cout_pad(a.Cout) / 64;
    p.bias = a.bias; p.Cout = a.Cout;
    p.gn_scale = a.gn_scale; p.gn_shift = a.gn_shift;
    p.chan_bias = a.chan_bias; p.chan_bias_stride = a.chan_bias_stride; p.residual = a.residual; p.relu = a.relu;
    p.out = a.out; p.stats = a.stats_out;
    p.nchunks = Cin / 8;
    const int pro = a.gn_scale == nullptr ? 0 : (a.gn_silu ? 2 : 1);
    {
        const bool ks_ok = p.nchunks % (4 * PWB_WAVES) == 0;
        if (a.tile_cfg == 35) SISIC_REQUIRE(ks_ok, "conv2d(pointwise bf16x3, K-split): tile_cfg 35 needs a multiple of 128 input channels");
        if (a.tile_cfg == 35 || (a.tile_cfg == 0 && ks_ok && p.HW <= 256 && a.Cout <= 256 && pwbk_on())) {
            if (pro == 2) return launch_pwbk<2>(ctx, p, Cin, s);
            if (pro == 1) return launch_pwbk<1>(ctx, p, Cin, s);
            return launch_pwbk<0>(ctx, p, Cin, s);
        }
    }
    if (a.tile_cfg == 34) SISIC_REQUIRE(pwbs_applicable(a), "conv2d(pointwise bf16x3, staged): tile_cfg 34 needs 384 .. 768 output channels and at most %d input channels", (150 * 1024) / 392);
    if (a.tile_cfg == 34 || (a.tile_cfg == 0 && pwbs_applicable(a) && (int64_t)a.B * (p.HW / 64) >= 128)) {
        if (pro == 2) return launch_pwbs<2>(ctx, p, Cin, s);
        if (pro == 1) return launch_pwbs<1>(ctx, p, Cin, s);
        return launch_pwbs<0>(ctx, p, Cin, s);
    }
    const bool wide = a.tile_cfg == 29 ? false : (a.tile_cfg == 30 ? true : (int64_t)a.B * (p.HW / 64) * (a.Cout / 64) >= 2048);
    if (wide) {
        if (pro == 2) return launch_pwb<2, 2>(ctx, p, Cin, s);
        if (pro == 1) return launch_pwb<1, 2>(ctx, p, Cin, s);
        return launch_pwb<0, 2>(ctx, p, Cin, s);
    }
    if (pro == 2) return launch_pwb<2, 1>(ctx, p, Cin, s);
    if (pro == 1) return launch_pwb<1, 1>(ctx, p, Cin, s);
    return launch_pwb<0, 1>(ctx, p, Cin, s);
}

}
```

synt_isic_amd/csrc/groupnorm.hip:

```cpp
#include "common.h"
#include "gn_merge.h"

namespace sisic {

constexpr int GN_THREADS = 256;

__device__ __forceinline__ float wave_sum(float v) {
#pragma unroll
    for (int o = 32; o > 0; o >>= 1) v += __shfl_xor(v, o, 64);
    return v;
}

__device__ __forceinline__ float block_sum(float v, float* red) {
    v = wave_sum(v);
    const int lane = threadIdx.x & 63, wave = threadIdx.x >> 6;
    __syncthreads();
    if (lane == 0) red[wave] = v;
    __syncthreads();
    float t = 0.0f;
#pragma unroll
    for (int w = 0; w < GN_THREADS / 64; ++w) t += red[w];
    return t;
}

__global__ void __launch_bounds__(GN_THREADS)
gn_stats_kernel(const float* __restrict__ in0, int c0, const float* __restrict__ in1, int c1, int HW, int groups,
                float eps, const float* __restrict__ gamma, const float* __restrict__ beta,
                float* __restrict__ scale, float* __restrict__ shift, int aligned16, float* __restrict__ mean_rstd) {
    __shared__ float red[GN_THREADS / 64];
    const int C = c0 + c1;
    const int cpg = C / groups;
    const int b = blockIdx.x / groups, g = blockIdx.x % groups;
    const int tid = threadIdx.x;
    const bool vec = aligned16 && (HW & 3) == 0;

    auto plane = [&](int c) -> const float* {
        return (c < c0) ? in0 + ((size_t)b * c0 + c) * HW : in1 + ((size_t)b * c1 + (c - c0)) * HW;
    };

    const float K = plane(g * cpg)[0];
    float s1 = 0.0f, s2 = 0.0f;
    for (int j = 0; j < cpg; ++j) {
        const float* src = plane(g * cpg + j);
        if (vec) {
            const float4* s4 = reinterpret_cast<const float4*>(src);
            const int n4 = HW / 4;
            int i = tid;
            for (; i + 3 * GN_THREADS < n4; i += 4 * GN_THREADS) {
                const float4 v0 = s4[i], v1 = s4[i + GN_THREADS], v2 = s4[i + 2 * GN_THREADS], v3 = s4[i + 3 * GN_THREADS];
                const float4 vv[4] = {v0, v1, v2, v3};
#pragma unroll
                for (int u = 0; u < 4; ++u) {
                    const float a = vv[u].x - K, bq = vv[u].y - K, c = vv[u].z - K, d = vv[u].w - K;
                    s1 += (a + bq) + (c + d);
                    s2 += (a * a + bq * bq) + (c * c + d * d);
                }
            }
            for (; i < n4; i += GN_THREADS) {
                const float4 v = s4[i];
                const float a = v.x - K, bq = v.y - K, c = v.z - K, d = v.w - K;
                s1 += (a + bq) + (c + d);
                s2 += (a * a + bq * bq) + (c * c + d * d);
            }
        } else {
            for (int i = tid; i < HW; i += GN_THREADS) {
                const float a = src[i] - K;
                s1 += a;
                s2 += a * a;
            }
        }
    }
    const float n = (float)cpg * (float)HW;
    const float m1 = block_sum(s1, red) / n;
    const float m2 = block_sum(s2, red) / n;
    const float mean = K + m1;
    const float var = fmaxf(m2 - m1 * m1, 0.0f);
    const float rstd = 1.0f / sqrtf(var + eps);
    if (mean_rstd && tid == 0) {
        mean_rstd[2 * (size_t)blockIdx.x] = mean;
        mean_rstd[2 * (size_t)blockIdx.x + 1] = rstd;
    }
    if (tid < cpg) {
        const int c = g * cpg + tid;
        const float sc = gamma[c] * rstd;
        scale[(size_t)b * C + c] = sc;
        shift[(size_t)b * C + c] = beta[c] - mean * sc;
    }
}

int launch_gn_stats(sisic_ctx* ctx, const float* in0, int c0, const float* in1, int c1, int B, int HW, int groups,
                    float eps, const float* gamma, const float* beta, float* scale, float* shift, hipStream_t s,
                    float* mean_rstd) {
    SISIC_REQUIRE(in0 && gamma && beta && scale && shift, "groupnorm_stats: null tensor");
    SISIC_REQUIRE((c1 == 0) == (in1 == nullptr), "groupnorm_stats: in1/c1 mismatch");
    const int C = c0 + c1;
    SISIC_REQUIRE(B > 0 && HW > 0 && groups > 0 && C % groups == 0, "groupnorm_stats: C=%d not divisible by groups=%d", C, groups);
    SISIC_REQUIRE(C / groups <= GN_THREADS, "groupnorm_stats: %d channels per group unsupported", C / groups);
    ProfileScope prof(ctx, s, PK_GN, 4.0 * B * C * HW + 8.0 * B * C, 0.0);
    const int aligned16 = ((reinterpret_cast<uintptr_t>(in0) | reinterpret_cast<uintptr_t>(in1)) & 15) == 0;
    hipLaunchKernelGGL(gn_stats_kernel, dim3(B * groups), dim3(GN_THREADS), 0, s, in0, c0, in1, c1, HW, groups, eps,
                       gamma, beta, scale, shift, aligned16, mean_rstd);
    SISIC_HIP(hipGetLastError());
    return SISIC_OK;
}

__device__ __forceinline__ double dpp_f64(double v, const int ctrl_sel) {
    const long long b = __double_as_longlong(v);
    int lo = (int)(b & 0xffffffffll), hi = (int)(b >> 32);
    switch (ctrl_sel) {
        case 0: lo = __builtin_amdgcn_update_dpp(0, lo, 0xB1, 0xf, 0xf, true); hi = __builtin_amdgcn_update_dpp(0, hi, 0xB1, 0xf, 0xf, true); break;
        case 1: lo = __builtin_amdgcn_update_dpp(0, lo, 0x4E, 0xf, 0xf, true); hi = __builtin_amdgcn_update_dpp(0, hi, 0x4E, 0xf, 0xf, true); break;
        case 2: lo = __builtin_amdgcn_update_dpp(0, lo, 0x141, 0xf, 0xf, true); hi = __builtin_amdgcn_update_dpp(0, hi, 0x141, 0xf, 0xf, true); break;
        default: lo = __builtin_amdgcn_update_dpp(0, lo, 0x140, 0xf, 0xf, true); hi = __builtin_amdgcn_update_dpp(0, hi, 0x140, 0xf, 0xf, true); break;
    }
    return __longlong_as_double(((long long)hi << 32) | (unsigned int)lo);
}
__device__ __forceinline__ double wave64_sum_f64(double v) {
    v += dpp_f64(v, 0);
    v += dpp_f64(v, 1);
    v += dpp_f64(v, 2);
    v += dpp_f64(v, 3);
    const long long b = __double_as_longlong(v);
    const int lo = (int)(b & 0xffffffffll), hi = (int)(b >> 32);
    double r[4];
#pragma unroll
    for (int i = 0; i < 4; ++i)
        r[i] = __longlong_as_double(((long long)__builtin_amdgcn_readlane(hi, 16 * i) << 32) |
                                    (unsigned int)__builtin_amdgcn_readlane(lo, 16 * i));
    return (r[0] + r[1]) + (r[2] + r[3]);
}

constexpr int GNF_WAVES = 4;
__global__ void __launch_bounds__(64 * GNF_WAVES) gn_finalize_kernel(const float4* __restrict__ st0, int c0, int slots0,
                                                         const float4* __restrict__ st1, int c1, int slots1,
                                                         int groups, int n_jobs, float eps, const float* __restrict__ gamma,
                                                         const float* __restrict__ beta, float* __restrict__ scale,
                                                         float* __restrict__ shift, float* __restrict__ mean_rstd) {
    const int C = c0 + c1, gs = C / groups;
    const int job = blockIdx.x * GNF_WAVES + (threadIdx.x >> 6);
    if (job >= n_jobs) return;
    const int b = job / groups, g = job % groups;
    const int lane = threadIdx.x & 63;
    const int ca = g * gs, cb = ca + gs;
    const int a0 = min(ca, c0), b0 = min(cb, c0);
    const int a1 = max(ca, c0) - c0, b1 = max(cb, c0) - c0;
    const float4* run0 = st0 + ((size_t)b * c0 + a0) * slots0;
    const int len0 = (b0 - a0) * slots0;
    const float4* run1 = st1 ? st1 + ((size_t)b * c1 + a1) * slots1 : nullptr;
    const int len1 = st1 ? (b1 - a1) * slots1 : 0;
    const float my_gamma = lane < gs ? gamma[ca + lane] : 0.0f, my_beta = lane < gs ? beta[ca + lane] : 0.0f;
    constexpr int KEEP = 4;
    float4 k0[KEEP], k1[KEEP];
    double n = 0.0, s1 = 0.0, m2 = 0.0;
#pragma unroll
    for (int j = 0; j < KEEP; ++j) {
        const int i = lane + 64 * j;
        k0[j] = i < len0 ? run0[i] : make_float4(0.f, 0.f, 0.f, 0.f);
        k1[j] = i < len1 ? run1[i] : make_float4(0.f, 0.f, 0.f, 0.f);
    }
#pragma unroll
    for (int j = 0; j < KEEP; ++j) {
        n += (double)k0[j].x + (double)k1[j].x;
        s1 += (double)k0[j].y + (double)k1[j].y;
        m2 += (double)k0[j].z + (double)k1[j].z;
    }
    for (int i = lane + 64 * KEEP; i < len0; i += 64) { const float4 v = run0[i]; n += v.x; s1 += v.y; m2 += v.z; }
    for (int i = lane + 64 * KEEP; i < len1; i += 64) { const float4 v = run1[i]; n += v.x; s1 += v.y; m2 += v.z; }
    n = wave64_sum_f64(n);
    s1 = wave64_sum_f64(s1);
    m2 = wave64_sum_f64(m2);
    const double mean = s1 / n;
    double between = 0.0;
    auto dev = [&](const float4 v) { between += gn_between_term(v.x, v.y, mean); };
#pragma unroll
    for (int j = 0; j < KEEP; ++j) { dev(k0[j]); dev(k1[j]); }
    for (int i = lane + 64 * KEEP; i < len0; i += 64) dev(run0[i]);
    for (int i = lane + 64 * KEEP; i < len1; i += 64) dev(run1[i]);
    between = wave64_sum_f64(between);
    float meanf, rstd;
    gn_mean_rstd(n, s1, m2, between, eps, meanf, rstd, mean);
    if (mean_rstd && lane == 0) {
        mean_rstd[2 * (size_t)job] = meanf;
        mean_rstd[2 * (size_t)job + 1] = rstd;
    }
    if (lane < gs) {
        float sc, sh;
        gn_affine(my_gamma, my_beta, meanf, rstd, sc, sh);
        scale[(size_t)b * C + ca + lane] = sc;
        shift[(size_t)b * C + ca + lane] = sh;
    }
    for (int cc = lane + 64; cc < gs; cc += 64) {
        const int c = ca + cc;
        float sc, sh;
        gn_affine(gamma[c], beta[c], meanf, rstd, sc, sh);
        scale[(size_t)b * C + c] = sc;
        shift[(size_t)b * C + c] = sh;
    }
}

int launch_gn_finalize(sisic_ctx* ctx, const float* st0, int c0, int slots0, const float* st1, int c1, int slots1, int B,
                       int HW, int groups, float eps, const float* gamma, const float* beta, float* scale, float* shift,
                       hipStream_t s, float* mean_rstd) {
    SISIC_REQUIRE(st0 && gamma && beta && scale && shift, "groupnorm_finalize: null tensor");
    SISIC_REQUIRE((c1 == 0) == (st1 == nullptr), "groupnorm_finalize: stats1/c1 mismatch");
    const int C = c0 + c1;
    SISIC_REQUIRE(B > 0 && HW > 0 && groups > 0 && c0 > 0 && C % groups == 0 && slots0 > 0 && (c1 == 0 || slots1 > 0),
                  "groupnorm_finalize: C=%d groups=%d slots=%d/%d", C, groups, slots0, slots1);
    (void)HW;
    ProfileScope prof(ctx, s, PK_GN, 16.0 * B * (c0 * (double)slots0 + c1 * (double)slots1) + 8.0 * B * C, 0.0);
    hipLaunchKernelGGL(gn_finalize_kernel, dim3(cdiv(B * groups, GNF_WAVES)), dim3(64 * GNF_WAVES), 0, s,
                       reinterpret_cast<const float4*>(st0), c0, slots0, reinterpret_cast<const float4*>(st1), c1, slots1, groups,
                       B * groups, eps, gamma, beta, scale, shift, mean_rstd);
    SISIC_HIP(hipGetLastError());
    return SISIC_OK;
}

}
```

synt_isic_amd/csrc/unet.cpp:

```cpp
#include <algorithm>
#include <cmath>
#include <cstdlib>
#include <cstring>
#include <map>
#include <memory>

#include "unet_internal.h"

using namespace sisic;

namespace {

void add_conv(sisic_unet* u, ConvW& c, const std::string& name, int cout, int cin, int k) {
    c.cout = cout; c.cin = cin; c.k = k;
    c.w_idx = u->add(name + ".weight", (int64_t)cout * cin * k * k);
    c.b_idx = u->add(name + ".bias", cout);
}
void add_norm(sisic_unet* u, NormW& n, const std::string& name, int c) {
    n.c = c;
    n.w_idx = u->add(name + ".weight", c);
    n.b_idx = u->add(name + ".bias", c);
}
void add_resnet(sisic_unet* u, ResnetW& r, const std::string& name, int cin, int cout) {
    r.cin = cin; r.cout = cout;
    add_norm(u, r.norm1, name + ".norm1", cin);
    add_conv(u, r.conv1, name + ".conv1", cout, cin, 3);
    r.temb_w_idx = u->add(name + ".time_emb_proj.weight", (int64_t)cout * u->hidden);
    r.temb_b_idx = u->add(name + ".time_emb_proj.bias", cout);
    r.temb_off = u->tproj_R;
    u->tproj_R += cout;
    add_norm(u, r.norm2, name + ".norm2", cout);
    add_conv(u, r.conv2, name + ".conv2", cout, cout, 3);
    if (cin != cout) add_conv(u, r.shortcut, name + ".conv_shortcut", cout, cin, 1);
    u->max_c = std::max(u->max_c, std::max(cin, cout));
}
void add_attn(sisic_unet* u, AttnW& a, const std::string& name, int c) {
    a.c = c;
    add_norm(u, a.norm, name + ".group_norm", c);
    a.q_w = u->add(name + ".to_q.weight", (int64_t)c * c); a.q_b = u->add(name + ".to_q.bias", c);
    a.k_w = u->add(name + ".to_k.weight", (int64_t)c * c); a.k_b = u->add(name + ".to_k.bias", c);
    a.v_w = u->add(name + ".to_v.weight", (int64_t)c * c); a.v_b = u->add(name + ".to_v.bias", c);
    add_conv(u, a.out, name + ".to_out.0", c, c, 1);
    u->max_c = std::max(u->max_c, c);
}

int describe(sisic_unet* u) {
    const sisic_unet_config& cfg = u->cfg;
    const int n = cfg.n_blocks;
    const int* boc = cfg.block_out_channels;
    u->hidden = 4 * boc[0];
    add_conv(u, u->conv_in, "conv_in", boc[0], cfg.in_channels, 3);
    u->temb_w1 = u->add("time_embedding.linear_1.weight", (int64_t)u->hidden * boc[0]);
    u->temb_b1 = u->add("time_embedding.linear_1.bias", u->hidden);
    u->temb_w2 = u->add("time_embedding.linear_2.weight", (int64_t)u->hidden * u->hidden);
    u->temb_b2 = u->add("time_embedding.linear_2.bias", u->hidden);

    u->down_res.resize(n); u->down_attn.resize(n); u->downsamplers.resize(n);
    int out_ch = boc[0];
    for (int i = 0; i < n; ++i) {
        const int in_ch = out_ch;
        out_ch = boc[i];
        u->down_res[i].resize(cfg.layers_per_block);
        if (cfg.down_attn[i]) u->down_attn[i].resize(cfg.layers_per_block);
        for (int j = 0; j < cfg.layers_per_block; ++j) {
            const std::string base = "down_blocks." + std::to_string(i);
            add_resnet(u, u->down_res[i][j], base + ".resnets." + std::to_string(j), j == 0 ? in_ch : out_ch, out_ch);
            if (cfg.down_attn[i]) add_attn(u, u->down_attn[i][j], base + ".attentions." + std::to_string(j), out_ch);
        }
        if (i != n - 1)
            add_conv(u, u->downsamplers[i], "down_blocks." + std::to_string(i) + ".downsamplers.0.conv", out_ch, out_ch, 3);
    }
    const int mid = boc[n - 1];
    add_resnet(u, u->mid_res[0], "mid_block.resnets.0", mid, mid);
    add_attn(u, u->mid_attn, "mid_block.attentions.0", mid);
    add_resnet(u, u->mid_res[1], "mid_block.resnets.1", mid, mid);

    u->up_res.resize(n); u->up_attn.resize(n); u->upsamplers.resize(n);
    out_ch = boc[n - 1];
    for (int i = 0; i < n; ++i) {
        const int prev_out = out_ch;
        out_ch = boc[n - 1 - i];
        const int in_ch = boc[n - 1 - std::min(i + 1, n - 1)];
        const int layers = cfg.layers_per_block + 1;
        u->up_res[i].resize(layers);
        if (cfg.up_attn[i]) u->up_attn[i].resize(layers);
        for (int j = 0; j < layers; ++j) {
            const int skip_ch = (j == layers - 1) ? in_ch : out_ch;
            const int res_in = (j == 0) ? prev_out : out_ch;
            const std::string base = "up_blocks." + std::to_string(i);
            add_resnet(u, u->up_res[i][j], base + ".resnets." + std::to_string(j), res_in + skip_ch, out_ch);
            if (cfg.up_attn[i]) add_attn(u, u->up_attn[i][j], base + ".attentions." + std::to_string(j), out_ch);
        }
        if (i != n - 1)
            add_conv(u, u->upsamplers[i], "up_blocks." + std::to_string(i) + ".upsamplers.0.conv", out_ch, out_ch, 3);
    }
    add_norm(u, u->norm_out, "conv_norm_out", boc[0]);
    add_conv(u, u->conv_out, "conv_out", cfg.out_channels, boc[0], 3);

    u->offsets.resize(u->names.size());
    size_t off = 0;
    for (size_t i = 0; i < u->names.size(); ++i) {
        u->offsets[i] = off;
        off += ((size_t)u->numels[i] + 3) / 4 * 4;
    }
    u->raw_floats = off;
    return SISIC_OK;
}

int dev_alloc(sisic_unet* u, size_t floats, float** out) {
    if (*out) return SISIC_OK;
    void* p = nullptr;
    SISIC_HIP(hipMalloc(&p, std::max<size_t>(floats, 4) * sizeof(float)));
    u->owned.push_back(static_cast<float*>(p));
    *out = static_cast<float*>(p);
    return SISIC_OK;
}

int prepare_conv(sisic_unet* u, ConvW& c, hipStream_t s) {
    if (c.k == 0) return SISIC_OK;
    SISIC_TRY(dev_alloc(u, (size_t)sisic_conv_packed_numel(c.cout, c.cin, c.k), &c.packed));
    SISIC_TRY(launch_conv_pack(u->ctx, u->rawp(c.w_idx), c.cout, c.cin, c.k, c.packed, s));
    c.bias = u->rawp(c.b_idx);
    if (c.k == 3 && !c.strided && c.cout > 4) {
        SISIC_TRY(dev_alloc(u, (size_t)winograd_packed_numel(c.cout, c.cin), &c.wino));
        SISIC_TRY(launch_winograd_pack(u->ctx, u->rawp(c.w_idx), c.cout, c.cin, c.wino, s));
    }
    return SISIC_OK;
}
void prepare_norm(sisic_unet* u, NormW& n) {
    n.gamma = u->rawp(n.w_idx);
    n.beta = u->rawp(n.b_idx);
}
int prepare_resnet(sisic_unet* u, ResnetW& r, hipStream_t s) {
    prepare_norm(u, r.norm1);
    prepare_norm(u, r.norm2);
    SISIC_TRY(prepare_conv(u, r.conv1, s));
    SISIC_TRY(prepare_conv(u, r.conv2, s));
    SISIC_TRY(prepare_conv(u, r.shortcut, s));
    SISIC_TRY(launch_transpose2d(u->ctx, u->rawp(r.temb_w_idx), r.cout, u->hidden, u->tproj_wt, u->tproj_R, r.temb_off, s));
    SISIC_HIP(hipMemcpyAsync(u->tproj_b + r.temb_off, u->rawp(r.temb_b_idx), (size_t)r.cout * sizeof(float), hipMemcpyDeviceToDevice, s));
    return SISIC_OK;
}
int prepare_attn(sisic_unet* u, AttnW& a, hipStream_t s) {
    prepare_norm(u, a.norm);
    const int c = a.c;
    SISIC_TRY(dev_alloc(u, (size_t)3 * c * c, &a.qkv_cat));
    float* cat = a.qkv_cat;
    const size_t wbytes = (size_t)c * c * sizeof(float);
    SISIC_HIP(hipMemcpyAsync(cat, u->rawp(a.q_w), wbytes, hipMemcpyDeviceToDevice, s));
    SISIC_HIP(hipMemcpyAsync(cat + (size_t)c * c, u->rawp(a.k_w), wbytes, hipMemcpyDeviceToDevice, s));
    SISIC_HIP(hipMemcpyAsync(cat + (size_t)2 * c * c, u->rawp(a.v_w), wbytes, hipMemcpyDeviceToDevice, s));
    SISIC_TRY(dev_alloc(u, (size_t)sisic_conv_packed_numel(3 * c, c, 1), &a.qkv_packed));
    SISIC_TRY(launch_conv_pack(u->ctx, cat, 3 * c, c, 1, a.qkv_packed, s));
    SISIC_TRY(dev_alloc(u, (size_t)3 * c, &a.qkv_bias));
    SISIC_HIP(hipMemcpyAsync(a.qkv_bias, u->rawp(a.q_b), c * sizeof(float), hipMemcpyDeviceToDevice, s));
    SISIC_HIP(hipMemcpyAsync(a.qkv_bias + c, u->rawp(a.k_b), c * sizeof(float), hipMemcpyDeviceToDevice, s));
    SISIC_HIP(hipMemcpyAsync(a.qkv_bias + 2 * c, u->rawp(a.v_b), c * sizeof(float), hipMemcpyDeviceToDevice, s));
    SISIC_TRY(prepare_conv(u, a.out, s));
    return SISIC_OK;
}

int prepare_all(sisic_unet* u, hipStream_t s) {
    const int nin = 2 * u->cfg.n_freqs;
    SISIC_TRY(dev_alloc(u, u->cfg.n_freqs, &u->d_freqs));
    SISIC_HIP(hipMemcpyAsync(u->d_freqs, u->freqs.data(), u->freqs.size() * sizeof(float), hipMemcpyHostToDevice, s));
    SISIC_TRY(dev_alloc(u, (size_t)nin * u->hidden, &u->w1t));
    SISIC_TRY(dev_alloc(u, (size_t)u->hidden * u->hidden, &u->w2t));
    SISIC_TRY(dev_alloc(u, (size_t)u->hidden * u->tproj_R, &u->tproj_wt));
    SISIC_TRY(dev_alloc(u, (size_t)u->tproj_R, &u->tproj_b));
    SISIC_TRY(launch_transpose2d(u->ctx, u->rawp(u->temb_w1), u->hidden, nin, u->w1t, u->hidden, 0, s));
    SISIC_TRY(launch_transpose2d(u->ctx, u->rawp(u->temb_w2), u->hidden, u->hidden, u->w2t, u->hidden, 0, s));
    SISIC_TRY(prepare_conv(u, u->conv_in, s));
    SISIC_TRY(prepare_conv(u, u->conv_out, s));
    prepare_norm(u, u->norm_out);
    for (auto& blk : u->down_res) for (auto& r : blk) SISIC_TRY(prepare_resnet(u, r, s));
    for (auto& blk : u->up_res) for (auto& r : blk) SISIC_TRY(prepare_resnet(u, r, s));
    for (auto& r : u->mid_res) SISIC_TRY(prepare_resnet(u, r, s));
    for (auto& blk : u->down_attn) for (auto& a : blk) SISIC_TRY(prepare_attn(u, a, s));
    for (auto& blk : u->up_attn) for (auto& a : blk) SISIC_TRY(prepare_attn(u, a, s));
    SISIC_TRY(prepare_attn(u, u->mid_attn, s));
    for (auto& c : u->downsamplers) {
        c.strided = true;
        SISIC_TRY(prepare_conv(u, c, s));
    }
    for (auto& c : u->upsamplers) SISIC_TRY(prepare_conv(u, c, s));
    return SISIC_OK;
}

void reset_conv(ConvW& c) { c.packed = c.wino = c.raw_t = c.packed_t = c.wino_t = nullptr; }
void reset_attn(AttnW& a) {
    a.qkv_cat = a.qkv_packed = a.qkv_bias = a.qkv_raw_t = a.qkv_packed_t = nullptr;
    reset_conv(a.out);
}
void reset_resnet(ResnetW& r) { reset_conv(r.conv1); reset_conv(r.conv2); reset_conv(r.shortcut); }
void reset_derived(sisic_unet* u) {
    if (u->train) u->train->repack_ready = false;
    u->d_freqs = u->w1t = u->w2t = u->tproj_wt = u->tproj_b = nullptr;
    reset_conv(u->conv_in); reset_conv(u->conv_out);
    for (auto& blk : u->down_res) for (auto& r : blk) reset_resnet(r);
    for (auto& blk : u->up_res) for (auto& r : blk) reset_resnet(r);
    for (auto& r : u->mid_res) reset_resnet(r);
    for (auto& blk : u->down_attn) for (auto& a : blk) reset_attn(a);
    for (auto& blk : u->up_attn) for (auto& a : blk) reset_attn(a);
    reset_attn(u->mid_attn);
    for (auto& c : u->downsamplers) reset_conv(c);
    for (auto& c : u->upsamplers) reset_conv(c);
}

void pool_put(sisic_unet* u, float* p);

void loop_graph_drop(sisic_unet* u) {
    if (u->loop_exec) (void)hipGraphExecDestroy(u->loop_exec);
    if (u->loop_graph) (void)hipGraphDestroy(u->loop_graph);
    u->loop_exec = nullptr; u->loop_graph = nullptr; u->loop_valid = false;
}

void tape_drop(sisic_unet* u, bool return_blocks) {
    TrainState* tr = u->train.get();
    if (!tr) return;
    if (return_blocks) {
        for (auto& b : tr->bufs) {
            if (b->p) pool_put(u, b->p);
            if (b->stats) pool_put(u, b->stats);
        }
        for (float* p : tr->grads_of_bufs) pool_put(u, p);
    }
    tr->bufs.clear();
    tr->grads_of_bufs.clear();
    tr->buf_grad.clear();
    tr->tape.clear();
    tr->has_tape = false;
}

void pool_release_all(sisic_unet* u) {
    loop_graph_drop(u);
    tape_drop(u, false);
    for (auto& b : u->pool) (void)hipFree(b.p);
    u->pool.clear();
}

int pool_get(sisic_unet* u, size_t floats, float** out) {
    const size_t bytes = floats * sizeof(float);
    for (auto& b : u->pool) {
        if (b.free_ && b.bytes == bytes) {
            b.free_ = false;
            *out = b.p;
            return SISIC_OK;
        }
    }
    void* p = nullptr;
    SISIC_HIP(hipMalloc(&p, bytes));
    u->pool.push_back({static_cast<float*>(p), bytes, false});
    *out = static_cast<float*>(p);
    return SISIC_OK;
}

void pool_put(sisic_unet* u, float* p) {
    for (auto& b : u->pool)
        if (b.p == p) { b.free_ = true; return; }
}

int grow(float** p, size_t* have, size_t want) {
    if (*have >= want) return SISIC_OK;
    if (*p) SISIC_HIP(hipFree(*p));
    *p = nullptr; *have = 0;
    void* q = nullptr;
    SISIC_HIP(hipMalloc(&q, want * sizeof(float)));
    *p = static_cast<float*>(q);
    *have = want;
    return SISIC_OK;
}

int ensure_rows(sisic_unet* u, size_t t_rows, size_t gn_rows) {
    SISIC_TRY(grow(&u->t_vals, &u->t_vals_cap, t_rows));
    SISIC_TRY(grow(&u->temb_act, &u->temb_act_cap, t_rows * u->hidden));
    SISIC_TRY(grow(&u->tproj, &u->tproj_cap, t_rows * u->tproj_R));
    SISIC_TRY(grow(&u->gn_scale, &u->gn_scale_cap, gn_rows * u->max_c));
    SISIC_TRY(grow(&u->gn_shift, &u->gn_shift_cap, gn_rows * u->max_c));
    SISIC_TRY(grow(&u->gn_scale2, &u->gn_scale2_cap, gn_rows * u->max_c));
    SISIC_TRY(grow(&u->gn_shift2, &u->gn_shift2_cap, gn_rows * u->max_c));
    return SISIC_OK;
}

int stage_upload(sisic_unet* u, const float* src, size_t n, float* dst, hipStream_t s) {
    if (u->stage_cap < n) {
        SISIC_HIP(hipDeviceSynchronize());
        if (u->stage_host) SISIC_HIP(hipHostFree(u->stage_host));
        u->stage_host = nullptr;
        const size_t cap = std::max<size_t>(n, 1024);
        void* p = nullptr;
        SISIC_HIP(hipHostMalloc(&p, cap * sisic_unet::STAGE_SLOTS * sizeof(float), hipHostMallocDefault));
        u->stage_host = static_cast<float*>(p);
        u->stage_cap = cap;
        for (int i = 0; i < sisic_unet::STAGE_SLOTS; ++i) u->stage_used[i] = false;
    }
    const int slot = (int)(u->stage_next++ % sisic_unet::STAGE_SLOTS);
    if (!u->stage_ev[slot]) SISIC_HIP(hipEventCreateWithFlags(&u->stage_ev[slot], hipEventDisableTiming));
    if (u->stage_used[slot]) SISIC_HIP(hipEventSynchronize(u->stage_ev[slot]));
    float* h = u->stage_host + (size_t)slot * u->stage_cap;
    std::memcpy(h, src, n * sizeof(float));
    SISIC_HIP(hipMemcpyAsync(dst, h, n * sizeof(float), hipMemcpyHostToDevice, s));
    SISIC_HIP(hipEventRecord(u->stage_ev[slot], s));
    u->stage_used[slot] = true;
    return SISIC_OK;
}

struct Fwd {
    sisic_unet* u;
    hipStream_t s;
    int B;
    const float* tproj;
    int tproj_stride;
    std::vector<std::unique_ptr<Buf>> bufs;
    TrainState* tr = nullptr;
    float* gsc = nullptr;
    float* gsh = nullptr;
    float* gmr = nullptr;
    const NormW* gnorm = nullptr;

    Buf* make(int C, int H, int W, int* rc) {
        auto b = std::make_unique<Buf>();
        b->C = C; b->H = H; b->W = W; b->refs = 1;
        *rc = pool_get(u, (size_t)B * C * H * W, &b->p);
        bufs.push_back(std::move(b));
        return bufs.back().get();
    }
    void release(Buf* b) {
        if (tr) return;
        if (b && --b->refs == 0 && b->p) {
            pool_put(u, b->p);
            b->p = nullptr;
            if (b->stats) { pool_put(u, b->stats); b->stats = nullptr; }
        }
    }

    int gn(const Buf* x, const Buf* skip, const NormW& n) {
        gsc = u->gn_scale; gsh = u->gn_shift; gmr = nullptr; gnorm = &n;
        if (!tr && !skip && x->fin_norm == static_cast<const void*>(&n)) {
            gsc = x->fin_scale; gsh = x->fin_shift;
            return SISIC_OK;
        }
        if (tr) {
            const int C = x->C + (skip ? skip->C : 0);
            SISIC_TRY(pool_get(u, (size_t)B * C, &gsc));
            SISIC_TRY(pool_get(u, (size_t)B * C, &gsh));
            SISIC_TRY(pool_get(u, (size_t)B * u->cfg.norm_groups * 2, &gmr));
            tr->grads_of_bufs.push_back(gsc); tr->grads_of_bufs.push_back(gsh); tr->grads_of_bufs.push_back(gmr);
        }
        if (x->stats && (!skip || skip->stats))
            return launch_gn_finalize(u->ctx, x->stats, x->C, x->slots, skip ? skip->stats : nullptr, skip ? skip->C : 0,
                                      skip ? skip->slots : 0, B, x->H * x->W, u->cfg.norm_groups, u->cfg.norm_eps,
                                      n.gamma, n.beta, gsc, gsh, s, gmr);
        return launch_gn_stats(u->ctx, x->p, x->C, skip ? skip->p : nullptr, skip ? skip->C : 0, B, x->H * x->W,
                               u->cfg.norm_groups, u->cfg.norm_eps, n.gamma, n.beta, gsc, gsh, s, gmr);
    }

    int conv(const ConvW& c, const float* in0, int c0, const float* in1, int c1, int H, int W, int stride, int ups,
             bool gn_prologue, bool silu, const float* chan_bias, const float* residual, float* out,
             Buf* normed_later = nullptr, Buf* xb = nullptr, Buf* skipb = nullptr, Buf* resb = nullptr, Buf* outb = nullptr,
             const AttnW* qkv_of = nullptr, const NormW* next_norm = nullptr) {
        sisic_conv_args a{};
        a.in0 = in0; a.c0 = c0; a.in1 = in1; a.c1 = c1;
        a.B = B; a.Hin = H; a.Win = W; a.upsample = ups; a.ksize = c.k; a.stride = stride;
        a.w_packed = c.packed; a.bias = c.bias; a.Cout = c.cout;
        a.w_winograd = (stride == 1 && u->use_winograd) ? c.wino : nullptr;
        if (gn_prologue) { a.gn_scale = gsc; a.gn_shift = gsh; a.gn_silu = silu ? 1 : 0; }
        a.chan_bias = chan_bias; a.chan_bias_stride = tproj_stride;
        a.residual = residual; a.out = out;
        if (u->latency_mode) {
            if (c.k == 3 && stride == 1 && !ups && a.w_winograd && c.cout > 4 && H >= 12 && W >= 12) a.tile_cfg = 79;
            else if (c.k == 1 && stride == 1) a.tile_cfg = 22;
            else if (c.k == 3 && stride == 2) a.tile_cfg = 18;
        }
        if (normed_later && u->fuse_gn) {
            const int slots = conv_stats_slots(a);
            if (slots > 0) {
                SISIC_TRY(pool_get(u, (size_t)B * c.cout * slots * 4, &normed_later->stats));
                normed_later->slots = slots;
                a.stats_out = normed_later->stats;
            }
        }
        if (normed_later && next_norm && u->fuse_gn && !tr) {
            a.fin_gamma = next_norm->gamma; a.fin_beta = next_norm->beta; a.fin_groups = u->cfg.norm_groups; a.fin_eps = u->cfg.norm_eps;
            const bool first_pair_busy = gn_prologue && gsc == u->gn_scale;
            a.fin_scale = first_pair_busy ? u->gn_scale2 : u->gn_scale;
            a.fin_shift = first_pair_busy ? u->gn_shift2 : u->gn_shift;
            if (conv_finalizes(a)) { normed_later->fin_norm = next_norm; normed_later->fin_scale = a.fin_scale; normed_later->fin_shift = a.fin_shift; }
            else { a.fin_gamma = nullptr; a.fin_beta = nullptr; a.fin_scale = nullptr; a.fin_shift = nullptr; }
        }
        if (tr) {
            TapeOp op;
            op.kind = TapeOp::CONV;
            op.w = c; op.qkv_of = qkv_of;
            op.in0 = xb; op.in1 = skipb; op.in0_ptr = in0; op.in1_ptr = in1;
            op.c0 = c0; op.c1 = c1; op.H = H; op.W = W; op.stride = stride; op.ups = ups;
            if (gn_prologue) { op.norm = gnorm; op.gn_scale = gsc; op.gn_shift = gsh; op.gn_mr = gmr; op.silu = silu; }
            op.temb_off = chan_bias ? (int)(chan_bias - tproj) : -1;
            op.residual = resb; op.out = outb; op.out_ptr = out;
            tr->tape.push_back(op);
        }
        return launch_conv2d(u->ctx, a, s);
    }

    int resnet(const ResnetW& r, const Buf* x, const Buf* skip, Buf** out, const NormW* next_norm = nullptr) {
        int rc = SISIC_OK;
        const int H = x->H, W = x->W;
        const int c1 = skip ? skip->C : 0;
        SISIC_REQUIRE(x->C + c1 == r.cin, "unet: resnet expects %d input channels, got %d", r.cin, x->C + c1);
        SISIC_TRY(gn(x, skip, r.norm1));
        Buf* h = make(r.cout, H, W, &rc); SISIC_TRY(rc);
        SISIC_TRY(conv(r.conv1, x->p, x->C, skip ? skip->p : nullptr, c1, H, W, 1, 0, true, true,
                       tproj + r.temb_off, nullptr, h->p, h, const_cast<Buf*>(x), const_cast<Buf*>(skip), nullptr, h, nullptr, &r.norm2));
        const float* residual = x->p;
        Buf* resb = const_cast<Buf*>(x);
        Buf* sc = nullptr;
        if (r.shortcut.k) {
            sc = make(r.cout, H, W, &rc); SISIC_TRY(rc);
            SISIC_TRY(conv(r.shortcut, x->p, x->C, skip ? skip->p : nullptr, c1, H, W, 1, 0, false, false, nullptr,
                           nullptr, sc->p, nullptr, const_cast<Buf*>(x), const_cast<Buf*>(skip), nullptr, sc));
            residual = sc->p;
            resb = sc;
        } else {
            SISIC_REQUIRE(c1 == 0 && x->C == r.cout, "unet: identity shortcut with mismatched channels");
        }
        SISIC_TRY(gn(h, nullptr, r.norm2));
        Buf* o = make(r.cout, H, W, &rc); SISIC_TRY(rc);
        SISIC_TRY(conv(r.conv2, h->p, r.cout, nullptr, 0, H, W, 1, 0, true, true, nullptr, residual, o->p, o, h, nullptr,
                       resb, o, nullptr, next_norm));
        release(h);
        release(sc);
        *out = o;
        return SISIC_OK;
    }

    int attention(const AttnW& a, const Buf* x, Buf** out) {
        int rc = SISIC_OK;
        const int H = x->H, W = x->W, N = H * W, C = a.c;
        SISIC_REQUIRE(x->C == C, "unet: attention channel mismatch");
        SISIC_TRY(gn(x, nullptr, a.norm));
        Buf* qkv = make(3 * C, H, W, &rc); SISIC_TRY(rc);
        ConvW cq; cq.cout = 3 * C; cq.cin = C; cq.k = 1; cq.packed = a.qkv_packed; cq.bias = a.qkv_bias;
        SISIC_TRY(conv(cq, x->p, C, nullptr, 0, H, W, 1, 0, true, false, nullptr, nullptr, qkv->p, nullptr,
                       const_cast<Buf*>(x), nullptr, nullptr, qkv, &a));
        Buf* o = make(C, H, W, &rc); SISIC_TRY(rc);
        SISIC_TRY(launch_attention(u->ctx, qkv->p, o->p, B, C, N, u->cfg.head_dim, s));
        if (tr) {
            TapeOp op;
            op.kind = TapeOp::ATTN;
            op.qkv = qkv; op.o = o; op.C = C; op.N = N;
            tr->tape.push_back(op);
        }
        release(qkv);
        Buf* y = make(C, H, W, &rc); SISIC_TRY(rc);
        SISIC_TRY(conv(a.out, o->p, C, nullptr, 0, H, W, 1, 0, false, false, nullptr, x->p, y->p, y, o, nullptr,
                       const_cast<Buf*>(x), y));
        release(o);
        *out = y;
        return SISIC_OK;
    }

    int run(const float* sample, float* out, int H, int W) {
        const sisic_unet_config& cfg = u->cfg;
        const int n = cfg.n_blocks;
        int rc = SISIC_OK;
        std::vector<Buf*> skips;

        Buf* x = make(u->conv_in.cout, H, W, &rc); SISIC_TRY(rc);
        SISIC_TRY(conv(u->conv_in, sample, cfg.in_channels, nullptr, 0, H, W, 1, 0, false, false, nullptr, nullptr, x->p, x,
                       nullptr, nullptr, nullptr, x));
        x->refs++;
        skips.push_back(x);

        for (int i = 0; i < n; ++i) {
            for (int j = 0; j < cfg.layers_per_block; ++j) {
                Buf* y = nullptr;
                const NormW* next = cfg.down_attn[i] ? &u->down_attn[i][j].norm
                                    : (j + 1 < cfg.layers_per_block ? &u->down_res[i][j + 1].norm1 : (i == n - 1 ? &u->mid_res[0].norm1 : nullptr));
                SISIC_TRY(resnet(u->down_res[i][j], x, nullptr, &y, next));
                release(x);
                x = y;
                if (cfg.down_attn[i]) {
                    SISIC_TRY(attention(u->down_attn[i][j], x, &y));
                    release(x);
                    x = y;
                }
                x->refs++;
                skips.push_back(x);
            }
            if (i != n - 1) {
                const int Ho = (x->H + 2 - 3) / 2 + 1, Wo = (x->W + 2 - 3) / 2 + 1;
                Buf* y = make(u->downsamplers[i].cout, Ho, Wo, &rc); SISIC_TRY(rc);
                SISIC_TRY(conv(u->downsamplers[i], x->p, x->C, nullptr, 0, x->H, x->W, 2, 0, false, false, nullptr, nullptr, y->p, y,
                               x, nullptr, nullptr, y));
                release(x);
                x = y;
                x->refs++;
                skips.push_back(x);
            }
        }

        {
            Buf* y = nullptr;
            SISIC_TRY(resnet(u->mid_res[0], x, nullptr, &y, &u->mid_attn.norm)); release(x); x = y;
            SISIC_TRY(attention(u->mid_attn, x, &y)); release(x); x = y;
            SISIC_TRY(resnet(u->mid_res[1], x, nullptr, &y)); release(x); x = y;
        }

        for (int i = 0; i < n; ++i) {
            const int layers = cfg.layers_per_block + 1;
            for (int j = 0; j < layers; ++j) {
                SISIC_REQUIRE(!skips.empty(), "unet: skip stack underflow");
                Buf* skip = skips.back();
                skips.pop_back();
                SISIC_REQUIRE(skip->H == x->H && skip->W == x->W, "unet: skip resolution %dx%d vs %dx%d (H and W must be divisible by %d)",
                              skip->H, skip->W, x->H, x->W, 1 << (n - 1));
                Buf* y = nullptr;
                SISIC_TRY(resnet(u->up_res[i][j], x, skip, &y, cfg.up_attn[i] ? &u->up_attn[i][j].norm : nullptr));
                release(x);
                release(skip);
                x = y;
                if (cfg.up_attn[i]) {
                    SISIC_TRY(attention(u->up_attn[i][j], x, &y));
                    release(x);
                    x = y;
                }
            }
            if (i != n - 1) {
                Buf* y = make(u->upsamplers[i].cout, 2 * x->H, 2 * x->W, &rc); SISIC_TRY(rc);
                SISIC_TRY(conv(u->upsamplers[i], x->p, x->C, nullptr, 0, x->H, x->W, 1, 1, false, false, nullptr, nullptr, y->p, y,
                               x, nullptr, nullptr, y));
                release(x);
                x = y;
            }
        }
        SISIC_REQUIRE(skips.empty(), "unet: skip stack not consumed");
        SISIC_REQUIRE(x->H == H && x->W == W, "unet: output resolution mismatch");
        SISIC_TRY(gn(x, nullptr, u->norm_out));
        SISIC_TRY(conv(u->conv_out, x->p, x->C, nullptr, 0, H, W, 1, 0, true, true, nullptr, nullptr, out, nullptr, x, nullptr,
                       nullptr, nullptr));
        release(x);
        return SISIC_OK;
    }
};

int check_shape(sisic_unet* u, int B, int H, int W) {
    SISIC_REQUIRE(u, "unet: null handle");
    if (!u->loaded) {
        set_error("unet: forward called before sisic_unet_load");
        return SISIC_ESTATE;
    }
    SISIC_HIP(hipSetDevice(u->ctx->device));
    const int div = 1 << (u->cfg.n_blocks - 1);
    SISIC_REQUIRE(B > 0 && H > 0 && W > 0 && H % div == 0 && W % div == 0,
                  "unet: sample %dx%dx%d unsupported (H and W must be positive multiples of %d)", B, H, W, div);
    if (u->ws_B != B || u->ws_H != H || u->ws_W != W) {
        SISIC_HIP(hipDeviceSynchronize());
        pool_release_all(u);
        u->ws_B = B; u->ws_H = H; u->ws_W = W;
    }
    return SISIC_OK;
}

int time_embed(sisic_unet* u, int rows, hipStream_t s) {
    SISIC_TRY(launch_temb_mlp(u->ctx, u->t_vals, rows, u->d_freqs, u->cfg.n_freqs, u->w1t, u->rawp(u->temb_b1), u->w2t,
                              u->rawp(u->temb_b2), u->hidden, u->temb_act, s));
    SISIC_TRY(launch_linear_t(u->ctx, u->temb_act, rows, u->hidden, u->tproj_wt, u->tproj_b, u->tproj_R, u->tproj, s));
    return SISIC_OK;
}

int run_forward(sisic_unet* u, const float* sample, const float* tproj, int tproj_stride, float* out, int B, int H,
                int W, hipStream_t s, TrainState* tr = nullptr) {
    Fwd f{u, s, B, tproj, tproj_stride, {}};
    f.tr = tr;
    f.gsc = u->gn_scale; f.gsh = u->gn_shift;
    const int rc = f.run(sample, out, H, W);
    if (tr && rc == SISIC_OK) {
        for (auto& b : f.bufs) tr->bufs.push_back(std::move(b));
        return rc;
    }
    for (auto& b : f.bufs) {
        if (b->p) pool_put(u, b->p);
        if (b->stats) pool_put(u, b->stats);
    }
    if (tr) tr->tape.clear();
    return rc;
}

}

namespace sisic {
int unet_pool_get(sisic_unet* u, size_t floats, float** out) { return pool_get(u, floats, out); }
void unet_release_tape(sisic_unet* u) { tape_drop(u, true); }
void unet_pool_put(sisic_unet* u, float* p) { pool_put(u, p); }
int unet_grow(float** p, size_t* have, size_t want) { return grow(p, have, want); }
int unet_check_shape(sisic_unet* u, int B, int H, int W) { return check_shape(u, B, H, W); }
int unet_ensure_rows(sisic_unet* u, size_t t_rows, size_t gn_rows) { return ensure_rows(u, t_rows, gn_rows); }
int unet_stage_upload(sisic_unet* u, const float* src, size_t n, float* dst, hipStream_t s) { return stage_upload(u, src, n, dst, s); }
int unet_prepare_all(sisic_unet* u, hipStream_t s) { return prepare_all(u, s); }
int unet_run_forward(sisic_unet* u, const float* sample, const float* tproj, int tproj_stride, float* out, int B, int H,
                     int W, hipStream_t s, TrainState* tape) {
    return run_forward(u, sample, tproj, tproj_stride, out, B, H, W, s, tape);
}
}

extern "C" {

int sisic_unet_create(sisic_ctx* ctx, const sisic_unet_config* cfg, sisic_unet** out) {
    SISIC_REQUIRE(ctx && cfg && out, "unet_create: null argument");
    *out = nullptr;
    SISIC_REQUIRE(cfg->n_blocks >= 1 && cfg->n_blocks <= 8, "unet_create: n_blocks %d", cfg->n_blocks);
    SISIC_REQUIRE(cfg->layers_per_block >= 1, "unet_create: layers_per_block");
    SISIC_REQUIRE(cfg->in_channels > 0 && cfg->out_channels > 0, "unet_create: channels");
    SISIC_REQUIRE(cfg->norm_groups > 0 && cfg->head_dim == 8, "unet_create: head_dim must be 8, groups > 0");
    SISIC_REQUIRE(cfg->freqs && cfg->n_freqs * 2 == cfg->block_out_channels[0], "unet_create: freqs table must hold block_out_channels[0]/2 entries");
    for (int i = 0; i < cfg->n_blocks; ++i)
        SISIC_REQUIRE(cfg->block_out_channels[i] > 0 && cfg->block_out_channels[i] % cfg->norm_groups == 0 &&
                          cfg->block_out_channels[i] % cfg->head_dim == 0,
                      "unet_create: block_out_channels[%d]=%d", i, cfg->block_out_channels[i]);
    auto* u = new sisic_unet();
    u->ctx = ctx;
    u->cfg = *cfg;
    u->freqs.assign(cfg->freqs, cfg->freqs + cfg->n_freqs);
    if (const char* e = std::getenv("SISIC_WINOGRAD")) u->use_winograd = std::atoi(e) != 0;
    if (const char* e = std::getenv("SISIC_FUSED_GN")) u->fuse_gn = std::atoi(e) != 0;
    if (const char* e = std::getenv("SISIC_GRAPH")) u->graph_mode = std::atoi(e) != 0 ? 1 : 0;
    u->cfg.freqs = nullptr;
    const int rc = describe(u);
    if (rc != SISIC_OK) { delete u; return rc; }
    *out = u;
    return SISIC_OK;
}

int sisic_unet_destroy(sisic_unet* u) {
    if (!u) return SISIC_OK;
    (void)sisic_unet_train_end(u);
    (void)hipDeviceSynchronize();
    pool_release_all(u);
    for (float* p : {u->x_work, u->loop_tables, u->tproj_cur, u->seeds_dev})
        if (p) (void)hipFree(p);
    if (u->loop_stream) (void)hipStreamDestroy(u->loop_stream);
    for (auto p : u->owned) (void)hipFree(p);
    for (float* p : {u->raw, u->t_vals, u->temb_act, u->tproj, u->gn_scale, u->gn_shift, u->gn_scale2, u->gn_shift2, u->eps_buf})
        if (p) (void)hipFree(p);
    if (u->stage_host) (void)hipHostFree(u->stage_host);
    for (auto e : u->stage_ev)
        if (e) (void)hipEventDestroy(e);
    delete u;
    return SISIC_OK;
}

int sisic_unet_set_latency_mode(sisic_unet* u, int on) {
    SISIC_REQUIRE(u, "set_latency_mode: null handle");
    u->latency_mode = on != 0;
    return SISIC_OK;
}

int sisic_unet_set_graph_mode(sisic_unet* u, int mode) {
    SISIC_REQUIRE(u && mode >= -1 && mode <= 1, "set_graph_mode: mode must be -1 (follow latency mode), 0 or 1");
    u->graph_mode = mode;
    return SISIC_OK;
}

int64_t sisic_unet_graph_builds(const sisic_unet* u) { return u ? u->loop_builds : 0; }

int64_t sisic_unet_workspace_bytes(const sisic_unet* u) {
    int64_t n = 0;
    if (u) for (const auto& b : u->pool) n += (int64_t)b.bytes;
    return n;
}

int sisic_unet_num_tensors(const sisic_unet* u) { return u ? (int)u->names.size() : 0; }

const char* sisic_unet_tensor_name(const sisic_unet* u, int i) {
    if (!u || i < 0 || i >= (int)u->names.size()) return nullptr;
    return u->names[i].c_str();
}

int sisic_unet_load(sisic_unet* u, int n, const char* const* names, const float* const* host_ptrs,
                    const int64_t* numels) {
    SISIC_REQUIRE(u && names && host_ptrs && numels, "unet_load: null argument");
    SISIC_REQUIRE(n == (int)u->names.size(), "unet_load: state dict has %d tensors, expected %d", n, (int)u->names.size());
    SISIC_HIP(hipSetDevice(u->ctx->device));
    if (!u->raw) {
        void* p = nullptr;
        SISIC_HIP(hipMalloc(&p, u->raw_floats * sizeof(float)));
        u->raw = static_cast<float*>(p);
    }
    SISIC_HIP(hipMemset(u->raw, 0, u->raw_floats * sizeof(float)));
    std::vector<char> seen(u->names.size(), 0);
    for (int i = 0; i < n; ++i) {
        SISIC_REQUIRE(names[i] && host_ptrs[i], "unet_load: entry %d is null", i);
        auto it = u->index.find(names[i]);
        SISIC_REQUIRE(it != u->index.end(), "unet_load: unexpected key '%s'", names[i]);
        const int idx = it->second;
        SISIC_REQUIRE(!seen[idx], "unet_load: duplicate key '%s'", names[i]);
        SISIC_REQUIRE(numels[i] == u->numels[idx], "unet_load: '%s' has %lld elements, expected %lld", names[i],
                      (long long)numels[i], (long long)u->numels[idx]);
        seen[idx] = 1;
        SISIC_HIP(hipMemcpy(u->raw + u->offsets[idx], host_ptrs[i], (size_t)numels[i] * sizeof(float), hipMemcpyHostToDevice));
    }
    SISIC_HIP(hipDeviceSynchronize());
    loop_graph_drop(u);
    for (auto p : u->owned) (void)hipFree(p);
    u->owned.clear();
    reset_derived(u);
    u->loaded = false;
    SISIC_TRY(prepare_all(u, nullptr));
    SISIC_HIP(hipDeviceSynchronize());
    u->loaded = true;
    return SISIC_OK;
}

int sisic_unet_forward(sisic_unet* u, const float* sample, const int64_t* timesteps, float* out, int B, int H, int W,
                       void* stream) {
    SISIC_REQUIRE(u && sample && timesteps && out, "unet_forward: null argument");
    hipStream_t s = static_cast<hipStream_t>(stream);
    SISIC_TRY(check_shape(u, B, H, W));
    SISIC_TRY(ensure_rows(u, (size_t)B, (size_t)B));
    std::vector<float> tv(B);
    bool uniform = true;
    for (int b = 0; b < B; ++b) {
        tv[b] = (float)timesteps[b];
        uniform = uniform && timesteps[b] == timesteps[0];
    }
    const int rows = uniform ? 1 : B;
    SISIC_TRY(stage_upload(u, tv.data(), (size_t)rows, u->t_vals, s));
    SISIC_TRY(time_embed(u, rows, s));
    return run_forward(u, sample, u->tproj, uniform ? 0 : u->tproj_R, out, B, H, W, s);
}

static int loop_step(sisic_unet* u, int B, int H, int W, size_t n, float clip, bool rng, hipStream_t s) {
    void* state = u->loop_tables;
    const float* coef_dev = u->loop_tables + 4;
    const int* zrow_dev = reinterpret_cast<const int*>(u->loop_tables + 4 + 5 * 1000);
    SISIC_TRY(launch_loop_select_row(u->ctx, u->tproj, u->tproj_R, state, u->tproj_cur, s));
    SISIC_TRY(run_forward(u, u->x_work, u->tproj_cur, 0, u->eps_buf, B, H, W, s));
    if (rng)
        SISIC_TRY(launch_ddpm_step_indexed_rng(u->ctx, u->eps_buf, u->x_work, (int64_t)n, (int64_t)(n / B), state, coef_dev,
                                               reinterpret_cast<const uint64_t*>(u->seeds_dev), clip, s));
    else
        SISIC_TRY(launch_ddpm_step_indexed(u->ctx, u->eps_buf, u->x_work, (int64_t)n, state, coef_dev, zrow_dev, clip, s));
    return launch_loop_advance(u->ctx, state, s);
}

static int sample_graph(sisic_unet* u, float* x, int B, int H, int W, int T, const float* coef, float clip, const float* noise,
                        bool rng, int step0, float* traj, const int* traj_row, const volatile int* cancel, int* steps_done,
                        hipStream_t caller) {
    const int C = u->cfg.in_channels;
    const size_t n = (size_t)B * C * H * W;
    SISIC_REQUIRE(T <= 1000, "sample: at most 1000 steps per call");
    tape_drop(u, true);
    hipStream_t s = caller;
    if (!s) {
        if (!u->loop_stream) SISIC_HIP(hipStreamCreate(&u->loop_stream));
        s = u->loop_stream;
    }
    SISIC_TRY(grow(&u->x_work, &u->x_work_cap, n));
    SISIC_TRY(grow(&u->tproj_cur, &u->tproj_cur_cap, (size_t)u->tproj_R));
    SISIC_TRY(grow(&u->loop_tables, &u->loop_tables_cap, (size_t)4 + 5 * 1000 + 1000));
    std::vector<float> tab(4 + 5 * 1000 + 1000, 0.0f);
    {
        const int first = 0, base = rng ? step0 : 0;
        std::memcpy(&tab[0], &first, sizeof(int));
        std::memcpy(&tab[1], &base, sizeof(int));
        std::memcpy(&tab[2], &noise, sizeof(noise));
        std::memcpy(&tab[4], coef, (size_t)T * 5 * sizeof(float));
        int* zr = reinterpret_cast<int*>(&tab[4 + 5 * 1000]);
        int zi = 0;
        for (int i = 0; i < T; ++i) zr[i] = (noise && coef[(size_t)i * 5 + 4] != 0.0f) ? zi++ : -1;
    }
    SISIC_TRY(stage_upload(u, tab.data(), tab.size(), u->loop_tables, s));
    SISIC_HIP(hipMemcpyAsync(u->x_work, x, n * sizeof(float), hipMemcpyDeviceToDevice, s));

    auto after_step = [&](int i) -> int {
        const int row = traj_row ? traj_row[i] : i;
        if (traj && row >= 0) SISIC_HIP(hipMemcpyAsync(traj + (size_t)row * n, u->x_work, n * sizeof(float), hipMemcpyDeviceToDevice, s));
        if (steps_done) *steps_done = i + 1;
        return SISIC_OK;
    };
    int rc = SISIC_OK;
    int i = 0;
    auto cancelled = [&](int at) -> bool {
        if (!cancel) return false;
        if ((at & 7) == 0) (void)hipStreamSynchronize(s);
        return *cancel != 0;
    };
    if (cancelled(0)) rc = SISIC_ECANCEL;
    auto reusable = [&]() -> bool {
        const uint64_t gen = u->ctx->scratch_generation.load();
        const void* ptrs[5] = {u->tproj, u->eps_buf, u->x_work, u->loop_tables, u->tproj_cur};
        bool ok = u->loop_valid && u->loop_key.B == B && u->loop_key.H == H && u->loop_key.W == W &&
                  u->loop_key.clip == clip && u->loop_key.s == s && u->loop_key.latency == u->latency_mode &&
                  u->loop_key.gen == gen && u->loop_key.rng == rng && (!rng || u->loop_key.seeds == u->seeds_dev);
        for (int k = 0; k < 5; ++k) ok = ok && u->loop_key.ptrs[k] == ptrs[k];
        return ok;
    };
    if (rc == SISIC_OK && !reusable()) {
        rc = loop_step(u, B, H, W, n, clip, rng, s);
        if (rc == SISIC_OK) rc = after_step(0);
        i = 1;
    }
    if (rc == SISIC_OK && i < T) {
        if (!reusable()) {
            const uint64_t gen = u->ctx->scratch_generation.load();
            const void* ptrs[5] = {u->tproj, u->eps_buf, u->x_work, u->loop_tables, u->tproj_cur};
            loop_graph_drop(u);
            SISIC_HIP(hipStreamBeginCapture(s, hipStreamCaptureModeRelaxed));
            const int crc = loop_step(u, B, H, W, n, clip, rng, s);
            hipGraph_t g = nullptr;
            const hipError_t e = hipStreamEndCapture(s, &g);
            if (crc != SISIC_OK || e != hipSuccess || !g) {
                if (g) (void)hipGraphDestroy(g);
                if (crc == SISIC_OK) set_error("sample: stream capture failed: %s", hipGetErrorString(e));
                return crc != SISIC_OK ? crc : SISIC_EHIP;
            }
            u->loop_graph = g;
            SISIC_HIP(hipGraphInstantiate(&u->loop_exec, g, nullptr, nullptr, 0));
            u->loop_key.B = B; u->loop_key.H = H; u->loop_key.W = W; u->loop_key.clip = clip; u->loop_key.s = s;
            u->loop_key.latency = u->latency_mode; u->loop_key.gen = gen;
            u->loop_key.rng = rng; u->loop_key.seeds = u->seeds_dev;
            for (int k = 0; k < 5; ++k) u->loop_key.ptrs[k] = ptrs[k];
            u->loop_valid = true;
            u->loop_builds += 1;
        }
        for (; i < T; ++i) {
            if (cancelled(i)) { rc = SISIC_ECANCEL; break; }
            SISIC_HIP(hipGraphLaunch(u->loop_exec, s));
            SISIC_TRY(after_step(i));
        }
    }
    SISIC_HIP(hipMemcpyAsync(x, u->x_work, n * sizeof(float), hipMemcpyDeviceToDevice, s));
    if (s != caller) SISIC_HIP(hipStreamSynchronize(s));
    if (rc == SISIC_ECANCEL) {
        SISIC_HIP(hipStreamSynchronize(s));
        set_error("sample: cancelled after %d of %d steps", steps_done ? *steps_done : i, T);
    }
    return rc;
}

int sisic_sample(sisic_unet* u, float* x, int B, int H, int W, int T, const int64_t* timesteps, const float* coef,
                 float clip, const float* noise, float* traj, uint8_t* out_u8, const volatile int* cancel,
                 int* steps_done, void* stream) {
    return sisic_sample_frames(u, x, B, H, W, T, timesteps, coef, clip, noise, traj, nullptr, out_u8, cancel, steps_done, stream);
}

static int sample_frames(sisic_unet* u, float* x, int B, int H, int W, int T, const int64_t* timesteps, const float* coef,
                         float clip, const float* noise, const uint64_t* seeds, int step0, float* traj, const int* traj_row,
                         uint8_t* out_u8, const volatile int* cancel, int* steps_done, void* stream) {
    SISIC_REQUIRE(u && x && timesteps && coef && T > 0, "sample: null argument");
    SISIC_REQUIRE(!traj_row || traj, "sample: traj_row without a trajectory buffer");
    if (traj_row)
        for (int i = 0; i < T; ++i) SISIC_REQUIRE(traj_row[i] >= -1, "sample: traj_row[%d] = %d (a row of traj, or -1)", i, traj_row[i]);
    hipStream_t s = static_cast<hipStream_t>(stream);
    if (steps_done) *steps_done = 0;
    SISIC_TRY(check_shape(u, B, H, W));
    SISIC_TRY(ensure_rows(u, (size_t)std::max(T, 1000), (size_t)B));
    const int C = u->cfg.in_channels;
    SISIC_REQUIRE(u->cfg.out_channels == C, "sample: in/out channels differ");
    const size_t n = (size_t)B * C * H * W;
    SISIC_TRY(grow(&u->eps_buf, &u->eps_floats, n));
    const bool rng = seeds != nullptr;
    if (rng) {
        SISIC_REQUIRE(step0 >= 0 && step0 <= INT32_MAX - T, "sample_rng: step0 %d", step0);
        static_assert(sizeof(uint64_t) == 2 * sizeof(float), "seeds are staged as pairs of floats");
        SISIC_TRY(grow(&u->seeds_dev, &u->seeds_cap, 2 * (size_t)std::max(B, 64)));
        SISIC_TRY(stage_upload(u, reinterpret_cast<const float*>(seeds), 2 * (size_t)B, u->seeds_dev, s));
    }

    std::vector<float> tv(T);
    for (int i = 0; i < T; ++i) tv[i] = (float)timesteps[i];
    SISIC_TRY(stage_upload(u, tv.data(), (size_t)T, u->t_vals, s));
    SISIC_TRY(time_embed(u, T, s));

    const bool use_graph = (u->graph_mode < 0 ? u->latency_mode : u->graph_mode != 0) && !u->ctx->profiling && T >= 4 && T <= 1000;
    if (use_graph) {
        if (!s) SISIC_HIP(hipStreamSynchronize(s));
        const int rc = sample_graph(u, x, B, H, W, T, coef, clip, noise, rng, step0, traj, traj_row, cancel, steps_done, s);
        if (rc != SISIC_OK) return rc;
        if (out_u8) SISIC_TRY(launch_denorm_u8(u->ctx, x, out_u8, B, C, H, W, s));
        return SISIC_OK;
    }

    size_t zi = 0;
    for (int i = 0; i < T; ++i) {
        if (cancel) {
            if ((i & 7) == 0) SISIC_HIP(hipStreamSynchronize(s));
            if (*cancel) {
                SISIC_HIP(hipStreamSynchronize(s));
                set_error("sample: cancelled after %d of %d steps", i, T);
                return SISIC_ECANCEL;
            }
        }
        SISIC_TRY(run_forward(u, x, u->tproj + (size_t)i * u->tproj_R, 0, u->eps_buf, B, H, W, s));
        const float* c = coef + (size_t)i * 5;
        const float* z = nullptr;
        if (noise && c[4] != 0.0f) z = noise + (zi++) * n;
        if (rng)
            SISIC_TRY(launch_ddpm_step_rng(u->ctx, u->eps_buf, x, x, (int64_t)n, (int64_t)(n / B),
                                           reinterpret_cast<const uint64_t*>(u->seeds_dev), (uint32_t)(step0 + i), c[0], c[1], c[2],
                                           c[3], c[4], clip, s));
        else
            SISIC_TRY(launch_ddpm_step(u->ctx, u->eps_buf, x, z, x, (int64_t)n, c[0], c[1], c[2], c[3], c[4], clip, s));
        const int row = traj_row ? traj_row[i] : i;
        if (traj && row >= 0) SISIC_HIP(hipMemcpyAsync(traj + (size_t)row * n, x, n * sizeof(float), hipMemcpyDeviceToDevice, s));
        if (steps_done) *steps_done = i + 1;
    }
    if (out_u8) SISIC_TRY(launch_denorm_u8(u->ctx, x, out_u8, B, C, H, W, s));
    return SISIC_OK;
}

int sisic_sample_frames(sisic_unet* u, float* x, int B, int H, int W, int T, const int64_t* timesteps, const float* coef,
                        float clip, const float* noise, float* traj, const int* traj_row, uint8_t* out_u8,
                        const volatile int* cancel, int* steps_done, void* stream) {
    return sample_frames(u, x, B, H, W, T, timesteps, coef, clip, noise, nullptr, 0, traj, traj_row, out_u8, cancel, steps_done,
                         stream);
}

int sisic_sample_frames_rng(sisic_unet* u, float* x, int B, int H, int W, int T, const int64_t* timesteps, const float* coef,
                            float clip, const uint64_t* seeds, int step0, float* traj, const int* traj_row, uint8_t* out_u8,
                            const volatile int* cancel, int* steps_done, void* stream) {
    SISIC_REQUIRE(seeds, "sample_rng: seeds is NULL");
    return sample_frames(u, x, B, H, W, T, timesteps, coef, clip, nullptr, seeds, step0, traj, traj_row, out_u8, cancel,
                         steps_done, stream);
}

}
```

Measured before the change: 12.19.

## Fold GroupNorm finalize into shortcut 1x1 conv launch as rider workgroups

In resnet blocks that have a 1x1 shortcut conv, the separate GroupNorm finalize kernel is removed. Its jobs now run as extra leading workgroups of the bf16x3 pointwise conv kernel, and the shortcut launch is reordered ahead of conv1 when that is legal. The aim is to cut per-step kernel launches and the serialization gaps between them across the T=1000 sampling loop. It adds template variants, a shared gn_finalize header and more complex ordering logic in unet.cpp. It only applies outside tape recording and only to prologue-free pointwise forms.

Result: no change. 12.24 (median of 6 runs) (+0.4%).

```diff
diff --git a/synt_isic_amd/csrc/common.h b/synt_isic_amd/csrc/common.h
--- a/synt_isic_amd/csrc/common.h
+++ b/synt_isic_amd/csrc/common.h
@@ -112,7 +112,10 @@
     return ksize == 1 ? 3 * first + first / 2 : first;
 }
 
-int launch_conv2d(sisic_ctx*, const sisic_conv_args& a, hipStream_t s);
+struct GnFinArgs;
+
+int launch_conv2d(sisic_ctx*, const sisic_conv_args& a, hipStream_t s, const GnFinArgs* rider = nullptr);
+bool conv_carries_rider(const sisic_conv_args& a);
 int launch_conv_smallcout(sisic_ctx*, const sisic_conv_args& a, hipStream_t s);
 int launch_score_head_bwd(sisic_ctx*, const float* logits, const float* fc_w, const float* act, float* g, int B, int C,
                           int HW, int n_classes, int target, hipStream_t s);
@@ -132,7 +135,8 @@
 int conv_pointwise_stats_slots(const sisic_conv_args& a);
 int launch_conv_pointwise(sisic_ctx*, const sisic_conv_args& a, hipStream_t s);
 bool conv_pointwise_bf3_applicable(const sisic_conv_args& a);
-int launch_conv_pointwise_bf3(sisic_ctx*, const sisic_conv_args& a, hipStream_t s);
+bool conv_pointwise_bf3_carries_rider(const sisic_conv_args& a);
+int launch_conv_pointwise_bf3(sisic_ctx*, const sisic_conv_args& a, hipStream_t s, const GnFinArgs* rider = nullptr);
 int launch_gn_finalize(sisic_ctx*, const float* st0, int c0, int slots0, const float* st1, int c1, int slots1, int B,
                        int HW, int groups, float eps, const float* gamma, const float* beta, float* scale, float* shift,
                        hipStream_t s, float* mean_rstd = nullptr);
diff --git a/synt_isic_amd/csrc/conv_mfma.hip b/synt_isic_amd/csrc/conv_mfma.hip
--- a/synt_isic_amd/csrc/conv_mfma.hip
+++ b/synt_isic_amd/csrc/conv_mfma.hip
@@ -428,7 +428,7 @@
     return SISIC_OK;
 }
 
-static int dispatch_conv2d(sisic_ctx* ctx, const sisic_conv_args& a, hipStream_t s, int* slots_query);
+static int dispatch_conv2d(sisic_ctx* ctx, const sisic_conv_args& a, hipStream_t s, int* slots_query, const GnFinArgs* rider = nullptr);
 
 static int winograd_cfg(const sisic_conv_args& a) {
     if (!(a.ksize == 3 && a.stride == 1 && a.w_winograd != nullptr && a.Cout > 4) || a.upsample == 2) return 0;
@@ -487,9 +487,16 @@
     return ((reinterpret_cast<uintptr_t>(a.residual) | reinterpret_cast<uintptr_t>(a.out) | reinterpret_cast<uintptr_t>(a.stats_out)) & 15) == 0;
 }
 
-int launch_conv2d(sisic_ctx* ctx, const sisic_conv_args& a, hipStream_t s) { return dispatch_conv2d(ctx, a, s, nullptr); }
-
-static int dispatch_conv2d(sisic_ctx* ctx, const sisic_conv_args& a, hipStream_t s, int* slots_query) {
+int launch_conv2d(sisic_ctx* ctx, const sisic_conv_args& a, hipStream_t s, const GnFinArgs* rider) { return dispatch_conv2d(ctx, a, s, nullptr, rider); }
+
+static bool pointwise_bf3_selected(const sisic_conv_args& a) {
+    static const bool pwb_on = [] { const char* e = std::getenv("SISIC_POINTWISE_BF16X3"); return !e || std::atoi(e) != 0; }();
+    const int cfg = a.tile_cfg;
+    return a.ksize == 1 && a.stride == 1 && ((cfg == 0 && pwb_on && conv_pointwise_bf3_applicable(a)) || (cfg >= 28 && cfg <= 30) || cfg == 34 || cfg == 35);
+}
+bool conv_carries_rider(const sisic_conv_args& a) { return pointwise_bf3_selected(a) && conv_pointwise_bf3_carries_rider(a); }
+
+static int dispatch_conv2d(sisic_ctx* ctx, const sisic_conv_args& a, hipStream_t s, int* slots_query, const GnFinArgs* rider) {
     SISIC_REQUIRE(a.in0 && a.w_packed && a.out, "conv2d: null tensor");
     SISIC_REQUIRE(a.B > 0 && a.Hin > 0 && a.Win > 0 && a.c0 > 0 && a.c1 >= 0 && a.Cout > 0, "conv2d: bad shape");
     SISIC_REQUIRE((a.c1 == 0) == (a.in1 == nullptr), "conv2d: in1/c1 mismatch");
@@ -498,6 +505,8 @@
     SISIC_REQUIRE(a.ksize != 7 || a.stride == 2, "conv2d: 7x7 is built for stride 2 only (the ResNet stem)");
     SISIC_REQUIRE(!(a.upsample && a.stride != 1), "conv2d: upsample with stride");
     SISIC_REQUIRE((a.gn_scale == nullptr) == (a.gn_shift == nullptr), "conv2d: gn_scale/gn_shift mismatch");
+    SISIC_REQUIRE(slots_query || !a.fin_gamma || conv_finalizes(a), "conv2d: fin_gamma given but sisic_conv_finalizes() is 0 for these arguments");
+    SISIC_REQUIRE(!rider || conv_carries_rider(a), "conv2d: this launch cannot carry a GroupNorm finalisation (conv_carries_rider)");
 
     ConvParams p{};
     p.in0 = a.in0; p.in1 = a.in1; p.c0 = a.c0; p.c1 = a.c1;
@@ -554,10 +563,9 @@
         p.Hin = 1; p.Win = a.Hin * a.Win; p.Hc = 1; p.Wc = p.Win; p.Hout = 1; p.Wout = p.Win; p.ups = 0;
         SISIC_REQUIRE(!a.upsample, "conv2d: 1x1 with upsample");
         static const bool pw_on = [] { const char* e = std::getenv("SISIC_POINTWISE"); return !e || std::atoi(e) != 0; }();
-        static const bool pwb_on = [] { const char* e = std::getenv("SISIC_POINTWISE_BF16X3"); return !e || std::atoi(e) != 0; }();
-        if ((cfg == 0 && pwb_on && conv_pointwise_bf3_applicable(a)) || (cfg >= 28 && cfg <= 30) || cfg == 34 || cfg == 35) {
+        if (pointwise_bf3_selected(a)) {
             if (slots_query) { *slots_query = conv_pointwise_stats_slots(a); return SISIC_OK; }
-            return launch_conv_pointwise_bf3(ctx, a, s);
+            return launch_conv_pointwise_bf3(ctx, a, s, rider);
         }
         if ((cfg == 0 && pw_on && conv_pointwise_applicable(a)) || cfg == 20) {
             if (slots_query) { *slots_query = conv_pointwise_stats_slots(a); return SISIC_OK; }
diff --git a/synt_isic_amd/csrc/conv_pointwise_bf3.hip b/synt_isic_amd/csrc/conv_pointwise_bf3.hip
--- a/synt_isic_amd/csrc/conv_pointwise_bf3.hip
+++ b/synt_isic_amd/csrc/conv_pointwise_bf3.hip
@@ -2,6 +2,7 @@
 #include <type_traits>
 
 #include "common.h"
+#include "gn_finalize.h"
 
 namespace sisic {
 
@@ -11,6 +12,8 @@
 typedef unsigned pwb_u2 __attribute__((ext_vector_type(2)));
 typedef float pwb_f2 __attribute__((ext_vector_type(2)));
 typedef float pwb_f4 __attribute__((ext_vector_type(4)));
+
+constexpr int PWB_WAVES = 4;
 
 struct PwbParams {
     const float* in0;
@@ -29,9 +32,11 @@
     float* out;
     float* stats;
     int n_px, n_co_items, nitems, nwg, nchunks;
+    GnFinArgs fin;
+    int rider_wgs;
 };
-
-constexpr int PWB_WAVES = 4;
+static_assert(PWB_WAVES == GNF_WAVES, "a rider workgroup is a workgroup of gn_finalize_kernel");
+
 
 __device__ __forceinline__ float pwb_half_wave_sum(float v) {
     v += __int_as_float(__builtin_amdgcn_update_dpp(0, __float_as_int(v), 0xB1, 0xf, 0xf, true));
@@ -49,12 +54,19 @@
 }
 __device__ __forceinline__ float pwb_silu(float v) { return v * __builtin_amdgcn_rcpf(1.0f + __expf(-v)); }
 
-template <int PRO, int NB>
+template <int PRO, int NB, bool RIDER = false>
 __global__ void __launch_bounds__(64 * PWB_WAVES, 4) conv_pwb_kernel(const PwbParams p) {
     extern __shared__ __attribute__((aligned(16))) float smem[];
+    if constexpr (RIDER) {
+        if ((int)blockIdx.x < p.rider_wgs) {
+            const int job = blockIdx.x * GNF_WAVES + (threadIdx.x >> 6);
+            if (job < p.fin.n_jobs) gn_finalize_job(job, threadIdx.x & 63, p.fin);
+            return;
+        }
+    }
     int wg;
     {
-        const int L = blockIdx.x, nwg = p.nwg;
+        const int L = RIDER ? blockIdx.x - p.rider_wgs : blockIdx.x, nwg = p.nwg;
         const int xcd = L & 7, slot = L >> 3, q = nwg >> 3, r = nwg & 7;
         wg = (xcd < r ? xcd * (q + 1) : r * (q + 1) + (xcd - r) * q) + slot;
     }
@@ -306,12 +318,19 @@
 #ifndef PWBK_VAR
 #define PWBK_VAR 0
 #endif
-template <int PRO>
+template <int PRO, bool RIDER = false>
 __global__ void __launch_bounds__(64 * PWB_WAVES, 4) conv_pwbk_kernel(const PwbParams p) {
     extern __shared__ __attribute__((aligned(16))) float smem[];
+    if constexpr (RIDER) {
+        if ((int)blockIdx.x < p.rider_wgs) {
+            const int job = blockIdx.x * GNF_WAVES + (threadIdx.x >> 6);
+            if (job < p.fin.n_jobs) gn_finalize_job(job, threadIdx.x & 63, p.fin);
+            return;
+        }
+    }
     int item;
     {
-        const int L = blockIdx.x, nwg = p.nwg;
+        const int L = RIDER ? blockIdx.x - p.rider_wgs : blockIdx.x, nwg = p.nwg;
         const int xcd = L & 7, slot = L >> 3, q = nwg >> 3, r = nwg & 7;
         item = (xcd < r ? xcd * (q + 1) : r * (q + 1) + (xcd - r) * q) + slot;
     }
@@ -682,6 +701,17 @@
     p.nitems = (int)nitems;
     p.nwg = p.nitems;
     const size_t lds = sizeof(float) * (size_t)(PWB_WAVES * 32 * 64 + (PRO ? 2 * Cin : 0));
+    if constexpr (PRO == 0) {
+        if (p.rider_wgs > 0) {
+            static std::atomic<uint64_t> opt_r{0};
+            auto kern_r = conv_pwbk_kernel<0, true>;
+            SISIC_TRY(ensure_dynamic_lds(ctx, reinterpret_cast<const void*>(kern_r), (int)lds, opt_r));
+            hipLaunchKernelGGL(kern_r, dim3(p.rider_wgs + p.nwg), dim3(64 * PWB_WAVES), lds, s, p);
+            SISIC_HIP(hipGetLastError());
+            return SISIC_OK;
+        }
+    }
+    SISIC_REQUIRE(p.rider_wgs == 0, "conv2d(pointwise bf16x3, K-split): a rider travels with the prologue-free form only");
     static std::atomic<uint64_t> opt{0};
     auto kern = conv_pwbk_kernel<PRO>;
     SISIC_TRY(ensure_dynamic_lds(ctx, reinterpret_cast<const void*>(kern), (int)lds, opt));
@@ -732,6 +762,14 @@
     p.nitems = (int)nitems;
     p.nwg = (int)((nitems + PWB_WAVES - 1) / PWB_WAVES);
     const size_t lds = PRO ? sizeof(float) * (size_t)(PWB_WAVES * 2 * Cin) : 0;
+    if constexpr (PRO == 0) {
+        if (p.rider_wgs > 0) {
+            hipLaunchKernelGGL((conv_pwb_kernel<0, NB, true>), dim3(p.rider_wgs + p.nwg), dim3(64 * PWB_WAVES), 0, s, p);
+            SISIC_HIP(hipGetLastError());
+            return SISIC_OK;
+        }
+    }
+    SISIC_REQUIRE(p.rider_wgs == 0, "conv2d(pointwise bf16x3): a rider travels with the prologue-free form only");
     static std::atomic<uint64_t> opt{0};
     auto kern = conv_pwb_kernel<PRO, NB>;
     SISIC_TRY(ensure_dynamic_lds(ctx, reinterpret_cast<const void*>(kern), (int)lds, opt));
@@ -740,7 +778,20 @@
     return SISIC_OK;
 }
 
-int launch_conv_pointwise_bf3(sisic_ctx* ctx, const sisic_conv_args& a, hipStream_t s) {
+static int pwb_form(const sisic_conv_args& a) {
+    const int HW = a.Hin * a.Win, nchunks = (a.c0 + a.c1) / 8;
+    const bool ks_ok = nchunks % (4 * PWB_WAVES) == 0;
+    if (a.tile_cfg == 35 || (a.tile_cfg == 0 && ks_ok && HW <= 256 && a.Cout <= 256 && pwbk_on())) return 0;
+    if (a.tile_cfg == 34 || (a.tile_cfg == 0 && pwbs_applicable(a) && (int64_t)a.B * (HW / 64) >= 128)) return 1;
+    const bool wide = a.tile_cfg == 29 ? false : (a.tile_cfg == 30 ? true : (int64_t)a.B * (HW / 64) * (a.Cout / 64) >= 2048);
+    return wide ? 2 : 3;
+}
+
+bool conv_pointwise_bf3_carries_rider(const sisic_conv_args& a) {
+    return conv_pointwise_bf3_applicable(a) && a.gn_scale == nullptr && pwb_form(a) != 1;
+}
+
+int launch_conv_pointwise_bf3(sisic_ctx* ctx, const sisic_conv_args& a, hipStream_t s, const GnFinArgs* rider) {
     SISIC_REQUIRE(conv_pointwise_bf3_applicable(a), "conv2d(pointwise bf16x3): shape not supported by tile_cfg 28");
     PwbParams p{};
     const int Cin = a.c0 + a.c1;
@@ -753,23 +804,28 @@
     p.out = a.out; p.stats = a.stats_out;
     p.nchunks = Cin / 8;
     const int pro = a.gn_scale == nullptr ? 0 : (a.gn_silu ? 2 : 1);
-    {
-        const bool ks_ok = p.nchunks % (4 * PWB_WAVES) == 0;
-        if (a.tile_cfg == 35) SISIC_REQUIRE(ks_ok, "conv2d(pointwise bf16x3, K-split): tile_cfg 35 needs a multiple of 128 input channels");
-        if (a.tile_cfg == 35 || (a.tile_cfg == 0 && ks_ok && p.HW <= 256 && a.Cout <= 256 && pwbk_on())) {
-            if (pro == 2) return launch_pwbk<2>(ctx, p, Cin, s);
-            if (pro == 1) return launch_pwbk<1>(ctx, p, Cin, s);
-            return launch_pwbk<0>(ctx, p, Cin, s);
-        }
-    }
-    if (a.tile_cfg == 34) SISIC_REQUIRE(pwbs_applicable(a), "conv2d(pointwise bf16x3, staged): tile_cfg 34 needs 384 .. 768 output channels and at most %d input channels", (150 * 1024) / 392);
-    if (a.tile_cfg == 34 || (a.tile_cfg == 0 && pwbs_applicable(a) && (int64_t)a.B * (p.HW / 64) >= 128)) {
+    const int form = pwb_form(a);
+    if (rider) {
+        SISIC_REQUIRE(conv_pointwise_bf3_carries_rider(a), "conv2d(pointwise bf16x3): this launch cannot carry a GroupNorm finalisation");
+        SISIC_REQUIRE(rider->st0 && rider->gamma && rider->beta && rider->scale && rider->shift && rider->n_jobs > 0 && rider->groups > 0 &&
+                          rider->c0 > 0 && (rider->c0 + rider->c1) % rider->groups == 0 && (rider->c1 == 0) == (rider->st1 == nullptr),
+                      "conv2d(pointwise bf16x3): incomplete GroupNorm finalisation rider");
+        p.fin = *rider;
+        p.rider_wgs = round_up(cdiv(rider->n_jobs, GNF_WAVES), 8);
+    }
+    if (form == 0) {
+        SISIC_REQUIRE(p.nchunks % (4 * PWB_WAVES) == 0, "conv2d(pointwise bf16x3, K-split): tile_cfg 35 needs a multiple of 128 input channels");
+        if (pro == 2) return launch_pwbk<2>(ctx, p, Cin, s);
+        if (pro == 1) return launch_pwbk<1>(ctx, p, Cin, s);
+        return launch_pwbk<0>(ctx, p, Cin, s);
+    }
+    if (form == 1) {
+        SISIC_REQUIRE(pwbs_applicable(a), "conv2d(pointwise bf16x3, staged): tile_cfg 34 needs 384 .. 768 output channels and at most %d input channels", (150 * 1024) / 392);
         if (pro == 2) return launch_pwbs<2>(ctx, p, Cin, s);
         if (pro == 1) return launch_pwbs<1>(ctx, p, Cin, s);
         return launch_pwbs<0>(ctx, p, Cin, s);
     }
-    const bool wide = a.tile_cfg == 29 ? false : (a.tile_cfg == 30 ? true : (int64_t)a.B * (p.HW / 64) * (a.Cout / 64) >= 2048);
-    if (wide) {
+    if (form == 2) {
         if (pro == 2) return launch_pwb<2, 2>(ctx, p, Cin, s);
         if (pro == 1) return launch_pwb<1, 2>(ctx, p, Cin, s);
         return launch_pwb<0, 2>(ctx, p, Cin, s);
diff --git a/synt_isic_amd/csrc/gn_finalize.h b/synt_isic_amd/csrc/gn_finalize.h
--- /dev/null
+++ b/synt_isic_amd/csrc/gn_finalize.h
@@ -0,0 +1,115 @@
+#pragma once
+
+#include <hip/hip_runtime.h>
+
+#include "gn_merge.h"
+
+namespace sisic {
+
+struct GnFinArgs {
+    const float4* st0;
+    const float4* st1;
+    int c0, slots0, c1, slots1;
+    int groups, n_jobs;
+    float eps;
+    const float* gamma;
+    const float* beta;
+    float* scale;
+    float* shift;
+    float* mean_rstd;
+};
+
+constexpr int GNF_WAVES = 4;
+
+__device__ __forceinline__ double dpp_f64(double v, const int ctrl_sel) {
+    const long long b = __double_as_longlong(v);
+    int lo = (int)(b & 0xffffffffll), hi = (int)(b >> 32);
+    switch (ctrl_sel) {
+        case 0: lo = __builtin_amdgcn_update_dpp(0, lo, 0xB1, 0xf, 0xf, true); hi = __builtin_amdgcn_update_dpp(0, hi, 0xB1, 0xf, 0xf, true); break;
+        case 1: lo = __builtin_amdgcn_update_dpp(0, lo, 0x4E, 0xf, 0xf, true); hi = __builtin_amdgcn_update_dpp(0, hi, 0x4E, 0xf, 0xf, true); break;
+        case 2: lo = __builtin_amdgcn_update_dpp(0, lo, 0x141, 0xf, 0xf, true); hi = __builtin_amdgcn_update_dpp(0, hi, 0x141, 0xf, 0xf, true); break;
+        default: lo = __builtin_amdgcn_update_dpp(0, lo, 0x140, 0xf, 0xf, true); hi = __builtin_amdgcn_update_dpp(0, hi, 0x140, 0xf, 0xf, true); break;
+    }
+    return __longlong_as_double(((long long)hi << 32) | (unsigned int)lo);
+}
+__device__ __forceinline__ double wave64_sum_f64(double v) {
+    v += dpp_f64(v, 0);
+    v += dpp_f64(v, 1);
+    v += dpp_f64(v, 2);
+    v += dpp_f64(v, 3);
+    const long long b = __double_as_longlong(v);
+    const int lo = (int)(b & 0xffffffffll), hi = (int)(b >> 32);
+    double r[4];
+#pragma unroll
+    for (int i = 0; i < 4; ++i)
+        r[i] = __longlong_as_double(((long long)__builtin_amdgcn_readlane(hi, 16 * i) << 32) |
+                                    (unsigned int)__builtin_amdgcn_readlane(lo, 16 * i));
+    return (r[0] + r[1]) + (r[2] + r[3]);
+}
+
+__device__ __forceinline__ void gn_finalize_job(const int job, const int lane, const GnFinArgs& f) {
+    const float4* __restrict__ st0 = f.st0;
+    const float4* __restrict__ st1 = f.st1;
+    const float* __restrict__ gamma = f.gamma;
+    const float* __restrict__ beta = f.beta;
+    const int c0 = f.c0, c1 = f.c1, slots0 = f.slots0, slots1 = f.slots1, groups = f.groups;
+    const int C = c0 + c1, gs = C / groups;
+    const int b = job / groups, g = job % groups;
+    const int ca = g * gs, cb = ca + gs;
+    const int a0 = min(ca, c0), b0 = min(cb, c0);
+    const int a1 = max(ca, c0) - c0, b1 = max(cb, c0) - c0;
+    const float4* run0 = st0 + ((size_t)b * c0 + a0) * slots0;
+    const int len0 = (b0 - a0) * slots0;
+    const float4* run1 = st1 ? st1 + ((size_t)b * c1 + a1) * slots1 : nullptr;
+    const int len1 = st1 ? (b1 - a1) * slots1 : 0;
+    const float my_gamma = lane < gs ? gamma[ca + lane] : 0.0f, my_beta = lane < gs ? beta[ca + lane] : 0.0f;
+    constexpr int KEEP = 4;
+    float4 k0[KEEP], k1[KEEP];
+    double n = 0.0, s1 = 0.0, m2 = 0.0;
+#pragma unroll
+    for (int j = 0; j < KEEP; ++j) {
+        const int i = lane + 64 * j;
+        k0[j] = i < len0 ? run0[i] : make_float4(0.f, 0.f, 0.f, 0.f);
+        k1[j] = i < len1 ? run1[i] : make_float4(0.f, 0.f, 0.f, 0.f);
+    }
+#pragma unroll
+    for (int j = 0; j < KEEP; ++j) {
+        n += (double)k0[j].x + (double)k1[j].x;
+        s1 += (double)k0[j].y + (double)k1[j].y;
+        m2 += (double)k0[j].z + (double)k1[j].z;
+    }
+    for (int i = lane + 64 * KEEP; i < len0; i += 64) { const float4 v = run0[i]; n += v.x; s1 += v.y; m2 += v.z; }
+    for (int i = lane + 64 * KEEP; i < len1; i += 64) { const float4 v = run1[i]; n += v.x; s1 += v.y; m2 += v.z; }
+    n = wave64_sum_f64(n);
+    s1 = wave64_sum_f64(s1);
+    m2 = wave64_sum_f64(m2);
+    const double mean = s1 / n;
+    double between = 0.0;
+    auto dev = [&](const float4 v) { between += gn_between_term(v.x, v.y, mean); };
+#pragma unroll
+    for (int j = 0; j < KEEP; ++j) { dev(k0[j]); dev(k1[j]); }
+    for (int i = lane + 64 * KEEP; i < len0; i += 64) dev(run0[i]);
+    for (int i = lane + 64 * KEEP; i < len1; i += 64) dev(run1[i]);
+    between = wave64_sum_f64(between);
+    float meanf, rstd;
+    gn_mean_rstd(n, s1, m2, between, f.eps, meanf, rstd, mean);
+    if (f.mean_rstd && lane == 0) {
+        f.mean_rstd[2 * (size_t)job] = meanf;
+        f.mean_rstd[2 * (size_t)job + 1] = rstd;
+    }
+    if (lane < gs) {
+        float sc, sh;
+        gn_affine(my_gamma, my_beta, meanf, rstd, sc, sh);
+        f.scale[(size_t)b * C + ca + lane] = sc;
+        f.shift[(size_t)b * C + ca + lane] = sh;
+    }
+    for (int cc = lane + 64; cc < gs; cc += 64) {
+        const int c = ca + cc;
+        float sc, sh;
+        gn_affine(gamma[c], beta[c], meanf, rstd, sc, sh);
+        f.scale[(size_t)b * C + c] = sc;
+        f.shift[(size_t)b * C + c] = sh;
+    }
+}
+
+}
diff --git a/synt_isic_amd/csrc/groupnorm.hip b/synt_isic_amd/csrc/groupnorm.hip
--- a/synt_isic_amd/csrc/groupnorm.hip
+++ b/synt_isic_amd/csrc/groupnorm.hip
@@ -1,5 +1,5 @@
 #include "common.h"
-#include "gn_merge.h"
+#include "gn_finalize.h"
 
 namespace sisic {
 
@@ -104,98 +104,10 @@
     return SISIC_OK;
 }
 
-__device__ __forceinline__ double dpp_f64(double v, const int ctrl_sel) {
-    const long long b = __double_as_longlong(v);
-    int lo = (int)(b & 0xffffffffll), hi = (int)(b >> 32);
-    switch (ctrl_sel) {
-        case 0: lo = __builtin_amdgcn_update_dpp(0, lo, 0xB1, 0xf, 0xf, true); hi = __builtin_amdgcn_update_dpp(0, hi, 0xB1, 0xf, 0xf, true); break;
-        case 1: lo = __builtin_amdgcn_update_dpp(0, lo, 0x4E, 0xf, 0xf, true); hi = __builtin_amdgcn_update_dpp(0, hi, 0x4E, 0xf, 0xf, true); break;
-        case 2: lo = __builtin_amdgcn_update_dpp(0, lo, 0x141, 0xf, 0xf, true); hi = __builtin_amdgcn_update_dpp(0, hi, 0x141, 0xf, 0xf, true); break;
-        default: lo = __builtin_amdgcn_update_dpp(0, lo, 0x140, 0xf, 0xf, true); hi = __builtin_amdgcn_update_dpp(0, hi, 0x140, 0xf, 0xf, true); break;
-    }
-    return __longlong_as_double(((long long)hi << 32) | (unsigned int)lo);
-}
-__device__ __forceinline__ double wave64_sum_f64(double v) {
-    v += dpp_f64(v, 0);
-    v += dpp_f64(v, 1);
-    v += dpp_f64(v, 2);
-    v += dpp_f64(v, 3);
-    const long long b = __double_as_longlong(v);
-    const int lo = (int)(b & 0xffffffffll), hi = (int)(b >> 32);
-    double r[4];
-#pragma unroll
-    for (int i = 0; i < 4; ++i)
-        r[i] = __longlong_as_double(((long long)__builtin_amdgcn_readlane(hi, 16 * i) << 32) |
-                                    (unsigned int)__builtin_amdgcn_readlane(lo, 16 * i));
-    return (r[0] + r[1]) + (r[2] + r[3]);
-}
-
-constexpr int GNF_WAVES = 4;
-__global__ void __launch_bounds__(64 * GNF_WAVES) gn_finalize_kernel(const float4* __restrict__ st0, int c0, int slots0,
-                                                         const float4* __restrict__ st1, int c1, int slots1,
-                                                         int groups, int n_jobs, float eps, const float* __restrict__ gamma,
-                                                         const float* __restrict__ beta, float* __restrict__ scale,
-                                                         float* __restrict__ shift, float* __restrict__ mean_rstd) {
-    const int C = c0 + c1, gs = C / groups;
+__global__ void __launch_bounds__(64 * GNF_WAVES) gn_finalize_kernel(const GnFinArgs f) {
     const int job = blockIdx.x * GNF_WAVES + (threadIdx.x >> 6);
-    if (job >= n_jobs) return;
-    const int b = job / groups, g = job % groups;
-    const int lane = threadIdx.x & 63;
-    const int ca = g * gs, cb = ca + gs;
-    const int a0 = min(ca, c0), b0 = min(cb, c0);
-    const int a1 = max(ca, c0) - c0, b1 = max(cb, c0) - c0;
-    const float4* run0 = st0 + ((size_t)b * c0 + a0) * slots0;
-    const int len0 = (b0 - a0) * slots0;
-    const float4* run1 = st1 ? st1 + ((size_t)b * c1 + a1) * slots1 : nullptr;
-    const int len1 = st1 ? (b1 - a1) * slots1 : 0;
-    const float my_gamma = lane < gs ? gamma[ca + lane] : 0.0f, my_beta = lane < gs ? beta[ca + lane] : 0.0f;
-    constexpr int KEEP = 4;
-    float4 k0[KEEP], k1[KEEP];
-    double n = 0.0, s1 = 0.0, m2 = 0.0;
-#pragma unroll
-    for (int j = 0; j < KEEP; ++j) {
-        const int i = lane + 64 * j;
-        k0[j] = i < len0 ? run0[i] : make_float4(0.f, 0.f, 0.f, 0.f);
-        k1[j] = i < len1 ? run1[i] : make_float4(0.f, 0.f, 0.f, 0.f);
-    }
-#pragma unroll
-    for (int j = 0; j < KEEP; ++j) {
-        n += (double)k0[j].x + (double)k1[j].x;
-        s1 += (double)k0[j].y + (double)k1[j].y;
-        m2 += (double)k0[j].z + (double)k1[j].z;
-    }
-    for (int i = lane + 64 * KEEP; i < len0; i += 64) { const float4 v = run0[i]; n += v.x; s1 += v.y; m2 += v.z; }
-    for (int i = lane + 64 * KEEP; i < len1; i += 64) { const float4 v = run1[i]; n += v.x; s1 += v.y; m2 += v.z; }
-    n = wave64_sum_f64(n);
-    s1 = wave64_sum_f64(s1);
-    m2 = wave64_sum_f64(m2);
-    const double mean = s1 / n;
-    double between = 0.0;
-    auto dev = [&](const float4 v) { between += gn_between_term(v.x, v.y, mean); };
-#pragma unroll
-    for (int j = 0; j < KEEP; ++j) { dev(k0[j]); dev(k1[j]); }
-    for (int i = lane + 64 * KEEP; i < len0; i += 64) dev(run0[i]);
-    for (int i = lane + 64 * KEEP; i < len1; i += 64) dev(run1[i]);
-    between = wave64_sum_f64(between);
-    float meanf, rstd;
-    gn_mean_rstd(n, s1, m2, between, eps, meanf, rstd, mean);
-    if (mean_rstd && lane == 0) {
-        mean_rstd[2 * (size_t)job] = meanf;
-        mean_rstd[2 * (size_t)job + 1] = rstd;
-    }
-    if (lane < gs) {
-        float sc, sh;
-        gn_affine(my_gamma, my_beta, meanf, rstd, sc, sh);
-        scale[(size_t)b * C + ca + lane] = sc;
-        shift[(size_t)b * C + ca + lane] = sh;
-    }
-    for (int cc = lane + 64; cc < gs; cc += 64) {
-        const int c = ca + cc;
-        float sc, sh;
-        gn_affine(gamma[c], beta[c], meanf, rstd, sc, sh);
-        scale[(size_t)b * C + c] = sc;
-        shift[(size_t)b * C + c] = sh;
-    }
+    if (job >= f.n_jobs) return;
+    gn_finalize_job(job, threadIdx.x & 63, f);
 }
 
 int launch_gn_finalize(sisic_ctx* ctx, const float* st0, int c0, int slots0, const float* st1, int c1, int slots1, int B,
@@ -208,9 +120,9 @@
                   "groupnorm_finalize: C=%d groups=%d slots=%d/%d", C, groups, slots0, slots1);
     (void)HW;
     ProfileScope prof(ctx, s, PK_GN, 16.0 * B * (c0 * (double)slots0 + c1 * (double)slots1) + 8.0 * B * C, 0.0);
-    hipLaunchKernelGGL(gn_finalize_kernel, dim3(cdiv(B * groups, GNF_WAVES)), dim3(64 * GNF_WAVES), 0, s,
-                       reinterpret_cast<const float4*>(st0), c0, slots0, reinterpret_cast<const float4*>(st1), c1, slots1, groups,
-                       B * groups, eps, gamma, beta, scale, shift, mean_rstd);
+    const GnFinArgs f{reinterpret_cast<const float4*>(st0), reinterpret_cast<const float4*>(st1), c0, slots0, c1, slots1, groups,
+                      B * groups, eps, gamma, beta, scale, shift, mean_rstd};
+    hipLaunchKernelGGL(gn_finalize_kernel, dim3(cdiv(B * groups, GNF_WAVES)), dim3(64 * GNF_WAVES), 0, s, f);
     SISIC_HIP(hipGetLastError());
     return SISIC_OK;
 }
diff --git a/synt_isic_amd/csrc/unet.cpp b/synt_isic_amd/csrc/unet.cpp
--- a/synt_isic_amd/csrc/unet.cpp
+++ b/synt_isic_amd/csrc/unet.cpp
@@ -6,6 +6,7 @@
 #include <memory>
 
 #include "unet_internal.h"
+#include "gn_finalize.h"
 
 using namespace sisic;
 
@@ -355,10 +356,24 @@
                                u->cfg.norm_groups, u->cfg.norm_eps, n.gamma, n.beta, gsc, gsh, s, gmr);
     }
 
+    bool gn_defer(const Buf* x, const Buf* skip, const NormW& n, GnFinArgs& f) {
+        if (tr || (!skip && x->fin_norm == static_cast<const void*>(&n))) return false;
+        if (!x->stats || (skip && !skip->stats)) return false;
+        gsc = u->gn_scale; gsh = u->gn_shift; gmr = nullptr; gnorm = &n;
+        f = GnFinArgs{reinterpret_cast<const float4*>(x->stats), reinterpret_cast<const float4*>(skip ? skip->stats : nullptr),
+                      x->C, x->slots, skip ? skip->C : 0, skip ? skip->slots : 0, u->cfg.norm_groups, B * u->cfg.norm_groups,
+                      u->cfg.norm_eps, n.gamma, n.beta, gsc, gsh, nullptr};
+        return true;
+    }
+    int gn_launch(const GnFinArgs& f, int HW) {
+        return launch_gn_finalize(u->ctx, reinterpret_cast<const float*>(f.st0), f.c0, f.slots0, reinterpret_cast<const float*>(f.st1),
+                                  f.c1, f.slots1, B, HW, f.groups, f.eps, f.gamma, f.beta, f.scale, f.shift, s, nullptr);
+    }
+
     int conv(const ConvW& c, const float* in0, int c0, const float* in1, int c1, int H, int W, int stride, int ups,
              bool gn_prologue, bool silu, const float* chan_bias, const float* residual, float* out,
              Buf* normed_later = nullptr, Buf* xb = nullptr, Buf* skipb = nullptr, Buf* resb = nullptr, Buf* outb = nullptr,
-             const AttnW* qkv_of = nullptr, const NormW* next_norm = nullptr) {
+             const AttnW* qkv_of = nullptr, const NormW* next_norm = nullptr, sisic_conv_args* hold = nullptr) {
         sisic_conv_args a{};
         a.in0 = in0; a.c0 = c0; a.in1 = in1; a.c1 = c1;
         a.B = B; a.Hin = H; a.Win = W; a.upsample = ups; a.ksize = c.k; a.stride = stride;
@@ -399,6 +414,7 @@
             op.residual = resb; op.out = outb; op.out_ptr = out;
             tr->tape.push_back(op);
         }
+        if (hold) { *hold = a; return SISIC_OK; }
         return launch_conv2d(u->ctx, a, s);
     }
 
@@ -407,23 +423,40 @@
         const int H = x->H, W = x->W;
         const int c1 = skip ? skip->C : 0;
         SISIC_REQUIRE(x->C + c1 == r.cin, "unet: resnet expects %d input channels, got %d", r.cin, x->C + c1);
-        SISIC_TRY(gn(x, skip, r.norm1));
+        static const bool rider_on = [] { const char* e = std::getenv("SISIC_GN_RIDER"); return !e || std::atoi(e) != 0; }();
+        const bool may_ride = rider_on && !tr && r.shortcut.k != 0;
+        GnFinArgs fin{};
+        const bool pend1 = may_ride && gn_defer(x, skip, r.norm1, fin);
+        if (!pend1) SISIC_TRY(gn(x, skip, r.norm1));
         Buf* h = make(r.cout, H, W, &rc); SISIC_TRY(rc);
+        sisic_conv_args a1{}, asc{};
         SISIC_TRY(conv(r.conv1, x->p, x->C, skip ? skip->p : nullptr, c1, H, W, 1, 0, true, true,
-                       tproj + r.temb_off, nullptr, h->p, h, const_cast<Buf*>(x), const_cast<Buf*>(skip), nullptr, h, nullptr, &r.norm2));
+                       tproj + r.temb_off, nullptr, h->p, h, const_cast<Buf*>(x), const_cast<Buf*>(skip), nullptr, h, nullptr, &r.norm2, &a1));
+        const bool conv1_fin = !tr && h->fin_norm == static_cast<const void*>(&r.norm2);
         const float* residual = x->p;
         Buf* resb = const_cast<Buf*>(x);
         Buf* sc = nullptr;
         if (r.shortcut.k) {
             sc = make(r.cout, H, W, &rc); SISIC_TRY(rc);
             SISIC_TRY(conv(r.shortcut, x->p, x->C, skip ? skip->p : nullptr, c1, H, W, 1, 0, false, false, nullptr,
-                           nullptr, sc->p, nullptr, const_cast<Buf*>(x), const_cast<Buf*>(skip), nullptr, sc));
+                           nullptr, sc->p, nullptr, const_cast<Buf*>(x), const_cast<Buf*>(skip), nullptr, sc, nullptr, nullptr, &asc));
             residual = sc->p;
             resb = sc;
         } else {
             SISIC_REQUIRE(c1 == 0 && x->C == r.cout, "unet: identity shortcut with mismatched channels");
         }
-        SISIC_TRY(gn(h, nullptr, r.norm2));
+        const bool carries = may_ride && conv_carries_rider(asc);
+        bool pend2 = false;
+        if (pend1 && conv1_fin && carries) {
+            SISIC_TRY(launch_conv2d(u->ctx, asc, s, &fin));
+            SISIC_TRY(launch_conv2d(u->ctx, a1, s));
+        } else {
+            if (pend1) SISIC_TRY(gn_launch(fin, H * W));
+            SISIC_TRY(launch_conv2d(u->ctx, a1, s));
+            pend2 = carries && !conv1_fin && gn_defer(h, nullptr, r.norm2, fin);
+            if (r.shortcut.k) SISIC_TRY(launch_conv2d(u->ctx, asc, s, pend2 ? &fin : nullptr));
+        }
+        if (!pend2) SISIC_TRY(gn(h, nullptr, r.norm2));
         Buf* o = make(r.cout, H, W, &rc); SISIC_TRY(rc);
         SISIC_TRY(conv(r.conv2, h->p, r.cout, nullptr, 0, H, W, 1, 0, true, true, nullptr, residual, o->p, o, h, nullptr,
                        resb, o, nullptr, next_norm));
```
